# Iheckzza/FeatureMatching

Hardware: AMD Instinct MI355X
Metric: image-pairs/sec at 640x480 (coarse corr + dual-softmax mutual-NN + fine window refinement) (higher is better)
Workload: dtype i8 screening + f32 exact; 1 GPU; 640x480 pair, C=256 @1/8 (L=S=4800), Cf=64 @1/2, 5x5 fine window, 'peaky' descriptors; launch=hipGraph replay, concurrent_streams=4, fine_maps_layout=nchw

## Files before the change

### featurematching_amd/_lib.py

```python
from __future__ import annotations

import ctypes as C
import os

_HERE = os.path.dirname(os.path.abspath(__file__))
LIB_PATH = os.path.join(_HERE, "lib", "libfmatch_hip.so")

FM_OK = 0
FM_F32, FM_F16, FM_BF16 = 0, 1, 2
FM_E_UNSUPPORTED = -3
FM_E_CAPACITY = -5
FM_E_CANDIDATES = -6
FM_E_RANGE = -7
FM_E_DENSE = -8
FM_E_INTERNAL = -9
FM_E_STEP = -10
FM_DEV_RANGE = 4
FM_DEV_ALL_DENSE = 256
FM_MODE_EXACT_SCREENING, FM_MODE_DENSE, FM_MODE_NO_CELL_MAPS, FM_MODE_EXACT_STEP, FM_MODE_STATS = 1, 2, 4, 8, 16
FM_MODE_FLAT = 32
FM_MODE_ALONE = 64
FM_LOSS_CROSS_ENTROPY, FM_LOSS_FOCAL = 0, 1
FM_LAYOUT_NCHW_PREPARED = 2

_lib = None

_p = C.c_void_p
_i = C.c_int
_f = C.c_float

SIGNATURES = {
    "fm_version": (_i, []),
    "fm_strerror": (C.c_char_p, [_i]),
    "fm_default_cand_slots": (_i, [_f]),
    "fm_coarse_workspace_bytes": (_i, [_i, _i, _i, _i, _i, C.POINTER(C.c_size_t)]),
    "fm_coarse_workspace_bytes_mode": (_i, [_i, _i, _i, _i, _i, _i, _i, C.POINTER(C.c_size_t)]),
    "fm_coarse_match": (_i, [_p, _p, _i, _i, _i, _i, _i, _i, _i, _i, _f, _f, _i, _f, _p, _p,
                             _p, C.c_size_t, _i, _i, _p, _p, _p, _p, _p, _p, _i, _p, _p, _p]),
    "fm_coarse_match_dtype": (_i, [_p, _p, _i, _i, _i, _i, _i, _i, _i, _i, _i, _f, _f, _i, _f, _p, _p,
                                   _p, C.c_size_t, _i, _i, _p, _p, _p, _p, _p, _p, _i, _p, _p, _p]),
    "fm_coarse_match_maps": (_i, [_p, _p, _i, _i, _i, _i, _i, _i, _i, _i, _i, _f, _f, _i, _f, _p, _p,
                                  _p, C.c_size_t, _i, _i, _p, _p, _p, _p, _p, _p, _i, _p, _p, _p, _i, _i, _i, _i, _p, _p]),
    "fm_coarse_workspace_bytes_auto": (_i, [_i, _i, _i, _i, _i, C.POINTER(C.c_size_t)]),
    "fm_coarse_match_auto": (_i, [_p, _p, _i, _i, _i, _i, _i, _i, _i, _i, _i, _f, _f, _i, _f, _p, _p,
                                  _p, C.c_size_t, _i, _i, _p, _p, _p, _p, _p, _p, _i, _p, _p,
                                  C.POINTER(C.c_int32), C.POINTER(C.c_int32), C.POINTER(C.c_int32), _p]),
    "fm_debug_coarse_layout": (_i, [_i, _i, _i, _i, _i, C.POINTER(C.c_int64), _i]),
    "fm_debug_launch_corr": (_i, [_p, _i, _i, _i, _i, _i, _f, _f, _i, _p]),
    "fm_debug_launch_screen": (_i, [_p, _p, _p, _i, _i, _i, _i, _i, _f, _f, _p]),
    "fm_debug_launch_prep": (_i, [_p, _p, _p, _i, _i, _i, _i, _i, _p]),
    "fm_debug_launch_prep_f16": (_i, [_p, _p, _p, _i, _i, _i, _i, _i, _i, _p]),
    "fm_debug_reset_counters": (_i, [_p, _i, _i, _i, _i, _i, _p]),
    "fm_debug_unit_cert": (_i, [_i]),
    "fm_debug_unit_cert_layout": (_i, [_i, _i, _i, _i, _i, C.POINTER(C.c_int64), _i]),
    "fm_read_count": (_i, [_p, _i, C.POINTER(C.c_int32), _p]),
    "fm_read_count_info": (_i, [_p, _i, C.POINTER(C.c_int32), C.POINTER(C.c_int32), _p]),
    "fm_debug_launch_flat": (_i, [_p, _p, _p, _i, _i, _i, _i, _i, _f, _f, _i, _p]),
    "fm_coarse_softmax_stats": (_i, [_p, _i, _i, _i, _i, _i, C.POINTER(_p), C.POINTER(_p), C.POINTER(_i), C.POINTER(_p),
                                     C.POINTER(_p), C.POINTER(_i)]),
    "fm_dual_softmax_conf_at": (_i, [_p, _p, _i, _i, _i, _i, _f, _p, _p, _i, _p, _p, _i, _p, _p, _p, _i, _p, _p]),
    "fm_dual_softmax_backward_workspace_bytes": (C.c_size_t, [_i, _i, _i, _i]),
    "fm_dual_softmax_backward": (_i, [_p, _p, _i, _i, _i, _i, _f, _p, _p, _i, _p, _p, _i, _p, _p, _p, _p, _i, _p, C.c_size_t, _p,
                                      _p, _p]),
    "fm_dual_softmax_backward_dense": (_i, [_p, _p, _i, _i, _i, _i, _f, _p, _p, _i, _p, _p, _i, _p, _p, C.c_size_t, _p, _p, _p]),
    "fm_coarse_loss_workspace_bytes": (C.c_size_t, [_i, _i, _i, _i, _i]),
    "fm_coarse_loss_forward": (_i, [_p, _p, _i, _i, _i, _i, _f, _p, _p, _i, _p, _p, _i, _i, _f, _f, _f, _f, _p, _p, _p, _i, _p,
                                    C.c_size_t, _p, _p]),
    "fm_coarse_loss_backward": (_i, [_p, _p, _i, _i, _i, _i, _f, _p, _p, _i, _p, _p, _i, _i, _f, _f, _f, _f, _p, _p, _p, _i, _p,
                                     C.c_size_t, _p, _p, _p, _p]),
    "fm_supervise_workspace_bytes": (C.c_size_t, [_i, _i, _i, _i]),
    "fm_supervise_matches": (_i, [_p, _p, _i, _i, _i, _i, _i, _f, _p, C.c_size_t, _p, _p, _p, _p, _p, _p, _p, _p, _p, _p, _i, _p,
                                  _p]),
    "fm_fine_loss_workspace_bytes": (C.c_size_t, [_i]),
    "fm_fine_loss_forward": (_i, [_p, _p, _i, _p, _p, _i, _p, _p, C.c_size_t, _p, _p]),
    "fm_fine_loss_backward": (_i, [_p, _p, _i, _p, _p, _i, _p, C.c_size_t, _p, _p, _p, _p]),
    "fm_gather_windows": (_i, [_p, _i, _i, _i, _i, _i, _i, _i, _i, _i, _p, _p, _p, _i, _p, _p]),
    "fm_gather_windows_dtype": (_i, [_p, _i, _i, _i, _i, _i, _i, _i, _i, _i, _i, _p, _p, _p, _i, _p, _p]),
    "fm_coarse_cell_maps": (_i, [_p, _i, _i, _i, _i, _i, C.POINTER(_p), C.POINTER(_i), C.POINTER(_p),
                                 C.POINTER(_p), C.POINTER(_i), C.POINTER(_p)]),
    "fm_gather_windows_cells": (_i, [_p, _i, _i, _i, _i, _i, _i, _i, _i, _i, _p, _i, _p, _p, _p, _p, _i, _p, _p]),
    "fm_merge_pack_weights": (_i, [_p, _i, _p, _p]),
    "fm_gather_merge_windows": (_i, [_p, _i, _i, _i, _i, _i, _i, _i, _i, _i, _p, _i, _p, _p, _p, _p, _p, _p, _i, _p, _p]),
    "fm_gather_windows_pair": (_i, [_p, _p, _i, _i, _i, _i, _i, _i, _i, _i, _i, _i, _i, _i, _i, _p, _i, _p, _p, _i, _p,
                                    _p, _p, _p, _p, _p, _p, _p, _i, _p, _p, _p]),
    "fm_gather_merge_windows_nhwc": (_i, [_p, _p, _i, _i, _i, _i, _i, _i, _i, _i, _i, _i, _i, _i, _i, _i, _p, _p, _p, _p, _p,
                                          _p, _p, _i, _p, _p, _p]),
    "fm_coarse_tf_packed_bytes": (C.c_size_t, [_i]),
    "fm_coarse_tf_workspace_bytes": (_i, [_i, _i, _i, C.POINTER(C.c_size_t)]),
    "fm_coarse_tf_pack_weights": (_i, [_p, _i, _p, _p]),
    "fm_coarse_transformer": (_i, [_p, _p, _i, _i, _i, _i, _i, _p, _i, _p, _p, C.c_size_t, _p, _p, _p]),
    "fm_coarse_transformer_masked": (_i, [_p, _p, _p, _p, _i, _i, _i, _i, _i, _p, _i, _p, _p, C.c_size_t, _p, _p, _p]),
    "fm_fine_tf_packed_bytes": (C.c_size_t, []),
    "fm_fine_tf_pack_weights": (_i, [_p, _p, _p, _p]),
    "fm_fine_transformer": (_i, [_p, _p, _i, _p, _i, _i, _p, _p, _p, _p]),
    "fm_fine_transformer_status": (_i, [_p, _p, _i, _p, _i, _i, _p, _p, _p, _p, _p]),
    "fm_fine_transformer_start": (_i, [_p, _p, _i, _p, _i, _i, _p, _p, _p, _p, _i, _p, _p]),
    "fm_epipolar_errors": (_i, [_p, _p, _i, _p, _p, _i, _i, _p, _p, _p, _f, _p, _p, _p, _p]),
    "fm_fine_match": (_i, [_p, _p, _i, _p, _i, _i, _p, _p, _p, _p, _f, _p, _p, _p]),
    "fm_fine_match_backward_workspace_bytes": (C.c_size_t, [_i, _i]),
    "fm_fine_match_backward": (_i, [_p, _p, _i, _p, _i, _i, _p, _p, _f, _p, _p, _p, C.c_size_t, _p, _p, _p, _p, _p]),
    "fm_gather_windows_backward_workspace_bytes": (C.c_size_t, [_i, _i, _i, _i]),
    "fm_gather_windows_backward": (_i, [_p, _p, _p, _p, _i, _i, _i, _i, _i, _i, _i, _i, _i, _i, _i, _p, C.c_size_t, _p,
                                        _p]),
    "fm_fine_maps_scratch_bytes": (C.c_size_t, [_i, _i, _i, _i, _i, _i, _i]),
    "fm_fine_maps_scratch_bytes_dtype": (C.c_size_t, [_i, _i, _i, _i, _i, _i, _i, _i]),
    "fm_fine_match_maps_dtype": (_i, [_p, _p, _i, _i, _i, _i, _i, _i, _i, _i, _i, _i, _i, _i, _i, _p, _p, _p, _p, _i, _p, _p,
                                      _p, _p, _f, _p, _p, _p, _p]),
    "fm_fine_match_maps": (_i, [_p, _p, _i, _i, _i, _i, _i, _i, _i, _i, _i, _i, _i, _i, _p, _p, _p, _p, _i, _p, _p,
                                _p, _p, _f, _p, _p, _p, _p]),
}


class FMatchError(RuntimeError):
    def __init__(self, status: int, where: str):
        self.status = status
        msg = load().fm_strerror(status).decode()
        super().__init__(f"{where}: {msg} (status {status})")


DEBUG_SIGNATURES = {k: v for k, v in SIGNATURES.items() if k.startswith("fm_debug_")}
SIGNATURES = {k: v for k, v in SIGNATURES.items() if not k.startswith("fm_debug_")}
ALL_SIGNATURES = {**SIGNATURES, **DEBUG_SIGNATURES}


def load(path=None):
    global _lib
    if _lib is None:
        lib_path = path or LIB_PATH
        if not os.path.exists(lib_path):
            raise RuntimeError(
                f"{lib_path} is missing: the HIP library is the product and has no fallback. "
                "Build it with `make -C featurematching_amd/csrc` (hipcc, --offload-arch=gfx950).")
        import torch
        lib = C.CDLL(lib_path)
        for name, (res, args) in ALL_SIGNATURES.items():
            fn = getattr(lib, name)
            fn.restype = res
            fn.argtypes = args
        _lib = lib
    elif path is not None and os.path.abspath(path) != os.path.abspath(getattr(_lib, '_name', '')):
        raise RuntimeError("the library is already loaded; load an experimental build before any other use")
    return _lib


def check(status: int, where: str) -> None:
    if status != FM_OK:
        raise FMatchError(status, where)
```

### featurematching_amd/csrc/api.hip

```cpp
#include <math.h>
#include <stdlib.h>

#include "fm_debug.h"
#include "fm_internal.h"

namespace fm {

int g_unit_cert = 0;

int choose_splits(int N, int panels, int tiles, int target) {
  const int wg = N * panels;
#ifdef FM_TUNE_ENV
  if (const char* e = getenv("FM_TARGET_WGS")) target = atoi(e) > 0 ? atoi(e) : 256;
#endif
  int s = target / (wg > 0 ? wg : 1);
  if (s < 1) s = 1;
  const int smax = tiles / 2 > 0 ? tiles / 2 : 1;
  if (s > smax) s = smax;
  if (s > 32) s = 32;
  return s;
}

static int choose_screen_chunks(int N, int Lp, int nunits, int* units_per_chunk, bool alone) {
  const long nrb = (long)N * (Lp / 32);
  const int cu = nrb * ((nunits + 63) / 64) >= 1024 ? 64 : (alone && nrb * ((nunits + 7) / 8) <= 8192 ? 8 : 32);
  *units_per_chunk = cu;
  return (nunits + cu - 1) / cu;
}

constexpr int kMaxPassTarget = 256;
constexpr int kMaxPassSlots = 512;

CoarseWs coarse_layout(int N, int L, int S, int C, int slots, bool alone) {
  CoarseWs w{};
  C = padded_channels(C);
  w.N = N; w.L = L; w.S = S; w.C = C; w.slots = slots;
  w.Lp = round_up(L, kPanelRows);
  w.Sp = round_up(S, kTileCols);
  w.panels = w.Lp / kPanelRows;
  w.tiles = w.Sp / kTileCols;
  w.splits = choose_splits(N, w.panels, w.tiles);
  {
    int target = N * w.panels >= kMaxPassSlots ? 10 * kMaxPassSlots : (alone ? kMaxPassSlots : kMaxPassTarget);
    if (target == kMaxPassTarget && w.tiles / choose_splits(N, w.panels, w.tiles, kMaxPassTarget) >= 32) target = kMaxPassSlots;
    w.splits0 = choose_splits(N, w.panels, w.tiles, target);
    w.top2 = N * w.panels < kMaxPassSlots && w.tiles / choose_splits(N, w.panels, w.tiles, kMaxPassTarget) < 32;
  }
#ifdef FM_TUNE_ENV
  if (const char* e = getenv("FM_TARGET_WGS0")) w.splits0 = choose_splits(N, w.panels, w.tiles, atoi(e) > 0 ? atoi(e) : kMaxPassTarget);
#endif
  w.splits_s = choose_screen_chunks(N, w.Lp, w.Sp / 32, &w.units_s, alone);
  const size_t rows = (size_t)N * w.Lp, cols = (size_t)N * w.Sp;
  const size_t nblk = (rows * slots + 255) / 256;
  size_t o = 0;
  auto take = [&](auto& r, size_t count) { r.at = o; o = align256(o + r.bytes(count)); };
  auto since = [&](size_t at) { return Span{at, o - at}; };
  take(w.cand.count, rows);
  take(w.ccand.count, cols);
  take(w.cand_b.count, rows);
  take(w.ccand_b.count, cols);
  take(w.dense_cnt, N);
  w.counters[0] = since(w.cand.count.at);
  take(w.cell0, rows);
  take(w.cell1, cols);
  take(w.ties0, kTieCap + 1);
  take(w.ties1, kTieCap + 1);
  w.reassign[0] = since(w.cell0.at);
  take(w.rowmax_u, rows);
  take(w.colmax_u, cols);
  take(w.blocktot, nblk);
  w.reassign[1] = since(w.blocktot.at);
  take(w.scalars, 1);
  w.reassign[2] = Span{w.scalars.at, sizeof(Scalars::flags)};
  w.counters[1] = Span{w.scalars.at, sizeof(Scalars)};
  w.prep_zero = since(w.cand.count.at);
  take(w.q0, rows * C); take(w.q1, cols * C);
  take(w.sigimg, (size_t)N * 2);
  take(w.imgstat, (size_t)N * 8);
  take(w.l1_0, rows); take(w.l1_1, cols);
  take(w.bstat0, rows / 32); take(w.bstat1, cols / 32);
  take(w.emarg, N);
  take(w.nmr, rows); take(w.nmc, cols);
  take(w.umax, rows / 32 * (cols / N / 32));
  take(w.cand.idx, rows * slots); take(w.cand.x, rows * slots);
  take(w.ccand.idx, cols * slots); take(w.ccand.x, cols * slots);
  take(w.thr_r, rows); take(w.thr_c, cols);
  take(w.wmaxb, rows / 32); take(w.cmaxu, cols / 32);
  take(w.tmin_r, rows / 32); take(w.tmin_c, cols / 32);
  take(w.umax2, rows / 32 * (cols / N / 32));
  take(w.upos, rows / 32 * (cols / N / 32));
  w.common_total = o;
  take(w.hi0, rows * C); take(w.lo0, rows * C);
  take(w.hi1, cols * C); take(w.lo1, cols * C);
  take(w.f16inv, N);
  take(w.rowB, rows * w.splits); take(w.colB, cols * w.panels);
  take(w.rsum, rows); take(w.csum, cols);
  take(w.nmr2, rows); take(w.nmc2, cols);
  take(w.cand_b.idx, rows * slots); take(w.cand_b.x, rows * slots);
  take(w.ccand_b.idx, cols * slots); take(w.ccand_b.x, cols * slots);
  w.total = o;
  return w;
}

}

using namespace fm;

extern "C" int fm_version(void) { return FM_VERSION; }

extern "C" const char* fm_strerror(int s) {
  switch (s) {
    case FM_OK: return "ok";
    case FM_E_NULL: return "required pointer is NULL";
    case FM_E_SHAPE: return "inconsistent or non-positive shape";
    case FM_E_UNSUPPORTED: return "unsupported configuration (C % 4 == 0 and C <= 256, Cf = 64, W in {5,7}, thr in (0,1))";
    case FM_E_WORKSPACE: return "workspace too small or not 256-byte aligned";
    case FM_E_CAPACITY: return "more matches than the output capacity";
    case FM_E_CANDIDATES: return "a coarse row or column exceeded its candidate slots (FM_MODE_EXACT_SCREENING, then more cand_slots)";
    case FM_E_RANGE: return "descriptor not finite or |x| >= 32768, or similarities of several thousand (screening margin >= 2^60)";
    case FM_E_DENSE: return "flat similarity in a sample: call again with FM_MODE_DENSE";
    case FM_E_INTERNAL: return "assignment kernel: bounded wait for predecessor workgroups ran out; call again";
    case FM_E_STEP: return "int8 screening step too small for a descriptor outside the sampled rows: call again with FM_MODE_EXACT_STEP";
    default: return s > 0 ? hipGetErrorString((hipError_t)s) : "unknown fmatch status";
  }
}

extern "C" int fm_default_cand_slots(float thr) {
  if (!(thr > 0.f)) return 64;
  int need = (int)ceilf(1.0f / thr) + 3;
  int s = 8;
  while (s < need && s < 64) s <<= 1;
  return s;
}

static float inv_ct_of(int C, float temperature) { return 1.0f / ((float)C * temperature); }

static bool valid_slots(int s) { return s >= 4 && s <= 64 && (s & (s - 1)) == 0; }

constexpr int kKnownModes = FM_MODE_DENSE | FM_MODE_EXACT_SCREENING | FM_MODE_NO_CELL_MAPS | FM_MODE_EXACT_STEP | FM_MODE_STATS |
                            FM_MODE_FLAT | FM_MODE_ALONE;

static int check_coarse_shape(int N, int L, int S, int C, int cand_slots) {
  if (N <= 0 || L <= 0 || S <= 0) return FM_E_SHAPE;
  if (!valid_channels(C) || !valid_slots(cand_slots)) return FM_E_UNSUPPORTED;
  return FM_OK;
}

static int checked_layout(bool have_ptrs, int N, int L, int S, int C, int cand_slots, CoarseWs* w) {
  if (!have_ptrs) return FM_E_NULL;
  if (const int bad = check_coarse_shape(N, L, S, C, cand_slots)) return bad;
  *w = coarse_layout(N, L, S, C, cand_slots);
  return FM_OK;
}

struct CoarsePlan {
  bool alone;
  bool exact_step;
  bool flat;
  bool allow_dead;
  bool prep_f16;
  int f16_force;
  bool dense;
  float list_cap;
  bool reduce;
  bool rescreen;
  bool exact_lists;
  bool conf;
  bool cell_maps;
  SelectFlags select() const { return {rescreen, dense, cell_maps, reduce}; }
  size_t workspace_bytes(const CoarseWs& w) const { return dense ? w.total : w.common_total; }
};

static CoarsePlan plan_coarse(int mode, bool conf, int cand_slots) {
  const bool all_rows = conf || (mode & FM_MODE_STATS) != 0;
  CoarsePlan p;
  p.alone = (mode & FM_MODE_ALONE) != 0;
  p.exact_step = (mode & FM_MODE_EXACT_STEP) != 0;
  p.flat = (mode & FM_MODE_FLAT) != 0 && !all_rows;
  p.allow_dead = !all_rows;
  p.dense = all_rows || (mode & (FM_MODE_DENSE | FM_MODE_EXACT_SCREENING | FM_MODE_FLAT)) != 0;
  p.prep_f16 = p.dense && !p.flat;
  p.f16_force = (mode & FM_MODE_EXACT_SCREENING) ? 1 : (conf ? 2 : 0);
  p.list_cap = conf ? 0.1f : 1.f;
  p.rescreen = (mode & FM_MODE_EXACT_SCREENING) != 0;
  p.reduce = p.rescreen || all_rows || (p.flat && cand_slots > 8);
  p.exact_lists = all_rows;
  p.conf = conf;
  p.cell_maps = (mode & FM_MODE_NO_CELL_MAPS) == 0;
  return p;
}

extern "C" int fm_coarse_workspace_bytes_mode(int N, int L, int S, int C, int cand_slots, int mode, int want_conf_matrix,
                                              size_t* bytes) {
  CoarseWs w;
  if (const int bad = checked_layout(bytes != nullptr, N, L, S, C, cand_slots, &w)) return bad;
  if (mode & ~kKnownModes) return FM_E_UNSUPPORTED;
  *bytes = plan_coarse(mode, want_conf_matrix != 0, cand_slots).workspace_bytes(w);
  return FM_OK;
}

extern "C" int fm_coarse_workspace_bytes(int N, int L, int S, int C, int cand_slots, size_t* bytes) {
  return fm_coarse_workspace_bytes_mode(N, L, S, C, cand_slots, FM_MODE_DENSE | FM_MODE_EXACT_SCREENING, 1, bytes);
}

extern "C" int fm_debug_coarse_layout(int N, int L, int S, int C, int cand_slots, int64_t* out, int n_out) {
  if (!out) return FM_E_NULL;
  if (n_out < 40) return FM_E_SHAPE;
  CoarseWs w;
  if (const int bad = checked_layout(true, N, L, S, C, cand_slots, &w)) return bad;
  const auto at = [](const auto& r) { return (int64_t)r.at; };
  const int64_t v[41] = {w.N, w.L, w.S, w.C, w.Lp, w.Sp, w.panels, w.tiles, w.splits, w.slots,
                         at(w.cand.count), at(w.ccand.count), at(w.scalars), at(w.blocktot), at(w.hi0), at(w.lo0),
                         at(w.hi1), at(w.lo1), at(w.q0), at(w.q1), at(w.sigimg), at(w.l1_0), at(w.nmr), at(w.nmr),
                         at(w.rowB), at(w.colB), at(w.nmr), at(w.nmc), at(w.rsum), at(w.csum), at(w.cand.idx),
                         at(w.cand.x), at(w.ccand.idx), at(w.umax), at(w.dense_cnt), at(w.rowmax_u), at(w.colmax_u),
                         w.splits_s, w.units_s, (int64_t)w.total, (int64_t)w.common_total};
  for (int i = 0; i < 40; ++i) out[i] = v[i];
  if (n_out > 40) out[40] = v[40];
  return FM_OK;
}

template <int K>
static hipError_t clear_spans(char* base, const Span (&spans)[K], hipStream_t st) {
  for (const Span& s : spans) {
    const hipError_t e = hipMemsetAsync(base + s.at, 0, s.bytes, st);
    if (e != hipSuccess) return e;
  }
  return hipSuccess;
}

static int coarse_match_impl(const CoarseCall& c, const MapCopyJob* job, bool resume) {
  if (!c.feat0 || !c.feat1 || !c.workspace || !c.d_count) return FM_E_NULL;
  if (c.in_dtype != FM_F32 && c.in_dtype != FM_F16 && c.in_dtype != FM_BF16) return FM_E_UNSUPPORTED;
  if (c.cap > 0 && (!c.b_ids || !c.i_ids || !c.j_ids || !c.mkpts0_c || !c.mkpts1_c || !c.mconf)) return FM_E_NULL;
  if (c.cap < 0 || c.L != c.h0c * c.w0c || c.S != c.h1c * c.w1c) return FM_E_SHAPE;
  if (const int bad = check_coarse_shape(c.N, c.L, c.S, c.C, c.cand_slots)) return bad;
  if (!(c.thr > 0.f) || !(c.thr < 1.f) || !(c.temperature > 0.f)) return FM_E_UNSUPPORTED;
  if (c.mode & ~kKnownModes) return FM_E_UNSUPPORTED;
  const CoarsePlan p = plan_coarse(c.mode, c.conf_matrix != nullptr, c.cand_slots);
  const CoarseWs w = coarse_layout(c.N, c.L, c.S, c.C, c.cand_slots, p.alone);
  if (c.workspace_bytes < p.workspace_bytes(w) || ((uintptr_t)c.workspace & 255)) return FM_E_WORKSPACE;
  char* base = (char*)c.workspace;
  hipStream_t st = (hipStream_t)c.stream;
  const float inv_ct = inv_ct_of(c.C, c.temperature);
  const float thr_list = fminf(c.thr, p.list_cap);
#define FM_TRY(call) do { const hipError_t e_ = (call); if (e_ != hipSuccess) return (int)e_; } while (0)
  if (!resume) {
    FM_TRY(launch_prep(c.feat0, c.feat1, c.in_dtype, c.C, w, base, p.exact_step, p.flat, st));
    FM_TRY(launch_max_i8(w, base, unit_cert_on(w, !p.dense), st));
    if (p.flat) FM_TRY(launch_stab(w, base, inv_ct, c.thr, p.allow_dead, st));
    else FM_TRY(launch_screen(c.feat0, c.feat1, c.in_dtype, c.C, w, base, inv_ct, c.thr, p.dense, p.allow_dead, st));
  } else {
    FM_TRY(clear_spans(base, w.reassign, st));
  }
  if (p.prep_f16) FM_TRY(launch_prep_f16(c.feat0, c.feat1, c.in_dtype, c.C, w, base, p.f16_force, st));
  if (p.dense) FM_TRY(launch_dense(w, base, inv_ct, thr_list, st));
  if (p.reduce) FM_TRY(launch_reduce(w, base, inv_ct, st));
  if (p.rescreen) FM_TRY(launch_dense(w, base, inv_ct, thr_list, st, nullptr, 1));
  if (p.exact_lists) FM_TRY(launch_exact_lists(w, base, inv_ct, c.feat0, c.feat1, c.in_dtype, c.C, st));
  if (p.conf) {
    FM_TRY(launch_dense(w, base, inv_ct, c.thr, st, c.conf_matrix));
    FM_TRY(launch_conf_patch(w, base, inv_ct, c.conf_matrix, st));
  }
#undef FM_TRY
  return (int)launch_select(w, base, c, inv_ct, p.select(), job);
}

extern "C" int fm_coarse_match(const float* feat0, const float* feat1, int N, int L, int S, int C, int h0c, int w0c,
                               int h1c, int w1c, float temperature, float thr, int border_rm, float scale_px,
                               const float* scale0, const float* scale1, void* workspace, size_t workspace_bytes,
                               int cand_slots, int mode, int64_t* b_ids, int64_t* i_ids, int64_t* j_ids,
                               float* mkpts0_c, float* mkpts1_c, float* mconf, int cap, int32_t* d_count,
                               float* conf_matrix, void* stream) {
  const CoarseCall c{feat0, feat1, FM_F32, N, L, S, C, h0c, w0c, h1c, w1c, temperature, thr, border_rm, scale_px, scale0, scale1,
                     workspace, workspace_bytes, cand_slots, mode, b_ids, i_ids, j_ids, mkpts0_c, mkpts1_c, mconf, cap,
                     d_count, conf_matrix, stream};
  return coarse_match_impl(c, nullptr, false);
}

extern "C" int fm_coarse_match_dtype(const void* feat0, const void* feat1, int in_dtype, int N, int L, int S, int C,
                                     int h0c, int w0c, int h1c, int w1c, float temperature, float thr, int border_rm,
                                     float scale_px, const float* scale0, const float* scale1, void* workspace,
                                     size_t workspace_bytes, int cand_slots, int mode, int64_t* b_ids,
                                     int64_t* i_ids, int64_t* j_ids, float* mkpts0_c, float* mkpts1_c, float* mconf,
                                     int cap, int32_t* d_count, float* conf_matrix, void* stream) {
  const CoarseCall c{feat0, feat1, in_dtype, N, L, S, C, h0c, w0c, h1c, w1c, temperature, thr, border_rm, scale_px, scale0,
                     scale1, workspace, workspace_bytes, cand_slots, mode, b_ids, i_ids, j_ids, mkpts0_c, mkpts1_c, mconf, cap,
                     d_count, conf_matrix, stream};
  return coarse_match_impl(c, nullptr, false);
}

extern "C" int fm_coarse_match_maps(const void* feat0, const void* feat1, int in_dtype, int N, int L, int S, int C,
                                    int h0c, int w0c, int h1c, int w1c, float temperature, float thr, int border_rm,
                                    float scale_px, const float* scale0, const float* scale1, void* workspace,
                                    size_t workspace_bytes, int cand_slots, int mode, int64_t* b_ids,
                                    int64_t* i_ids, int64_t* j_ids, float* mkpts0_c, float* mkpts1_c, float* mconf,
                                    int cap, int32_t* d_count, float* conf_matrix, const float* feat_f1, int Nf, int Cf,
                                    int Hf1, int Wf1, void* scratch1, void* stream) {
  if (!feat_f1 || !scratch1) return FM_E_NULL;
  if (Nf <= 0 || Hf1 <= 0 || Wf1 <= 0) return FM_E_SHAPE;
  if (Cf != 64) return FM_E_UNSUPPORTED;
  if (((uintptr_t)scratch1 & 15) || ((uintptr_t)feat_f1 & 15)) return FM_E_WORKSPACE;
  const MapCopyJob job{feat_f1, (float*)scratch1, Nf, Hf1, Wf1};
  const CoarseCall c{feat0, feat1, in_dtype, N, L, S, C, h0c, w0c, h1c, w1c, temperature, thr, border_rm, scale_px, scale0,
                     scale1, workspace, workspace_bytes, cand_slots, mode, b_ids, i_ids, j_ids, mkpts0_c, mkpts1_c, mconf, cap,
                     d_count, conf_matrix, stream};
  return coarse_match_impl(c, &job, false);
}

constexpr int kAutoDataModes = FM_MODE_DENSE | FM_MODE_EXACT_SCREENING | FM_MODE_EXACT_STEP | FM_MODE_FLAT;

extern "C" int fm_coarse_workspace_bytes_auto(int N, int L, int S, int C, int max_cand_slots, size_t* bytes) {
  if (max_cand_slots == 0) max_cand_slots = 64;
  return fm_coarse_workspace_bytes(N, L, S, C, max_cand_slots, bytes);
}

extern "C" int fm_coarse_match_auto(const void* feat0, const void* feat1, int in_dtype, int N, int L, int S, int C,
                                    int h0c, int w0c, int h1c, int w1c, float temperature, float thr, int border_rm,
                                    float scale_px, const float* scale0, const float* scale1, void* workspace,
                                    size_t workspace_bytes, int max_cand_slots, int mode, int64_t* b_ids, int64_t* i_ids,
                                    int64_t* j_ids, float* mkpts0_c, float* mkpts1_c, float* mconf, int cap,
                                    int32_t* d_count, float* conf_matrix, int32_t* hint_io, int32_t* m_out,
                                    int32_t* info_out, void* stream) {
  if (!m_out) return FM_E_NULL;
  if (max_cand_slots == 0) max_cand_slots = 64;
  if (!valid_slots(max_cand_slots)) return FM_E_UNSUPPORTED;
  if (mode & ~kKnownModes) return FM_E_UNSUPPORTED;
  if (!(thr > 0.f) || !(thr < 1.f)) return FM_E_UNSUPPORTED;
  const int slots0 = fm_default_cand_slots(thr) < max_cand_slots ? fm_default_cand_slots(thr) : max_cand_slots;
  const int fixed = mode & ~kAutoDataModes;
  const bool full_stats = conf_matrix != nullptr || (mode & FM_MODE_STATS) != 0;
  int cur = mode & kAutoDataModes;
  if (full_stats) cur |= FM_MODE_EXACT_SCREENING;
  int slots = slots0;
  if (conf_matrix && slots < 16 && max_cand_slots >= 16) slots = 16;
  const int slots_start = slots;
  if (hint_io && *hint_io) {
    cur |= *hint_io & kAutoDataModes;
    const int hs = (*hint_io >> 8) & 0xff;
    if (valid_slots(hs) && hs <= max_cand_slots && hs > slots) slots = hs;
  }
  bool tried_wide = slots > slots0, retried_internal = false;
  int st = FM_OK;
  int32_t m = 0, info = 0;
  int attempts = 0;
  CoarseCall c{feat0, feat1, in_dtype, N, L, S, C, h0c, w0c, h1c, w1c, temperature, thr, border_rm, scale_px, scale0, scale1,
               workspace, workspace_bytes, slots, mode, b_ids, i_ids, j_ids, mkpts0_c, mkpts1_c, mconf, cap, d_count,
               conf_matrix, stream};
  for (int attempt = 0; attempt < 10; ++attempt) {
    ++attempts;
    const int call_mode = fixed | cur | ((cur & FM_MODE_FLAT) ? FM_MODE_DENSE : 0);
    c.cand_slots = slots; c.mode = call_mode;
    st = coarse_match_impl(c, nullptr, false);
    if (st != FM_OK) return st;
    st = fm_read_count_info(d_count, cap, &m, &info, stream);
    if (st == FM_E_DENSE && !(cur & FM_MODE_DENSE) && !conf_matrix && !(mode & FM_MODE_STATS)) {
      cur |= FM_MODE_DENSE;
      if ((info & ~FM_DEV_ALL_DENSE) != FM_DEV_DENSE) continue;
      c.mode = fixed | cur;
      st = coarse_match_impl(c, nullptr, true);
      if (st != FM_OK) return st;
      st = fm_read_count_info(d_count, cap, &m, &info, stream);
    }
    if (st == FM_OK) break;
    if (st == FM_E_STEP && !(cur & FM_MODE_EXACT_STEP)) { cur |= FM_MODE_EXACT_STEP; continue; }
    if (st == FM_E_DENSE && !(cur & FM_MODE_DENSE)) { cur |= FM_MODE_DENSE; continue; }
    if (st == FM_E_CANDIDATES && (cur & FM_MODE_DENSE) && !tried_wide && slots < 16 && max_cand_slots >= 16 &&
        !(cur & FM_MODE_EXACT_SCREENING)) {
      slots = 16; cur |= FM_MODE_EXACT_STEP; tried_wide = true;
      continue;
    }
    if (st == FM_E_CANDIDATES && !(cur & FM_MODE_EXACT_SCREENING)) {
      if (tried_wide) slots = slots0;
      cur |= FM_MODE_EXACT_SCREENING | FM_MODE_DENSE;
      continue;
    }
    if (st == FM_E_CANDIDATES && slots < max_cand_slots) { slots *= 2; continue; }
    if (st == FM_E_INTERNAL && !retried_internal) { retried_internal = true; continue; }
    break;
  }
  *m_out = m;
  if (info_out) *info_out = info;
  if (hint_io && (st == FM_OK || st == FM_E_CAPACITY)) {
    int learnt = cur & kAutoDataModes;
    if (full_stats) learnt &= ~FM_MODE_EXACT_SCREENING | (mode & FM_MODE_EXACT_SCREENING);
    if ((learnt & FM_MODE_DENSE) && !full_stats) {
      if (info & FM_DEV_ALL_DENSE) learnt |= FM_MODE_FLAT; else learnt &= ~FM_MODE_FLAT;
    }
    *hint_io = learnt | (slots != slots_start ? slots << 8 : 0) | (slots << 16) | (attempts << 24);
  }
  return st;
}

extern "C" int fm_coarse_cell_maps(void* workspace, int N, int L, int S, int C, int cand_slots, int32_t** cell0,
                                   int* pitch0, int32_t** ties0, int32_t** cell1, int* pitch1, int32_t** ties1) {
  CoarseWs w;
  if (const int bad = checked_layout(workspace && cell0 && cell1 && pitch0 && pitch1 && ties0 && ties1, N, L, S, C,
                                     cand_slots, &w))
    return bad;
  *cell0 = w.cell0.in(workspace); *pitch0 = w.Lp; *ties0 = w.ties0.in(workspace);
  *cell1 = w.cell1.in(workspace); *pitch1 = w.Sp; *ties1 = w.ties1.in(workspace);
  return FM_OK;
}

extern "C" int fm_coarse_softmax_stats(void* workspace, int N, int L, int S, int C, int cand_slots, const float** nm_r,
                                       const float** sum_r, int* pitch_r, const float** nm_c, const float** sum_c,
                                       int* pitch_c) {
  CoarseWs w;
  if (const int bad = checked_layout(workspace && nm_r && sum_r && pitch_r && nm_c && sum_c && pitch_c, N, L, S, C,
                                     cand_slots, &w))
    return bad;
  *nm_r = w.nmr.in(workspace); *sum_r = w.rsum.in(workspace); *pitch_r = w.Lp;
  *nm_c = w.nmc.in(workspace); *sum_c = w.csum.in(workspace); *pitch_c = w.Sp;
  return FM_OK;
}

extern "C" int fm_debug_launch_corr(void* workspace, int N, int L, int S, int C, int cand_slots, float temperature,
                                    float thr, int mode, void* stream) {
  CoarseWs w;
  if (const int bad = checked_layout(workspace, N, L, S, C, cand_slots, &w)) return bad;
  if (mode < 0 || mode > 2) return FM_E_UNSUPPORTED;
  hipStream_t st = (hipStream_t)stream;
  if (mode == 0) return (int)launch_max_i8(w, (char*)workspace, unit_cert_on(w), st);
  if (mode == 1) return (int)launch_dense(w, (char*)workspace, inv_ct_of(C, temperature), thr, st);
  return (int)launch_dense(w, (char*)workspace, inv_ct_of(C, temperature), thr, st, nullptr, 1);
}

extern "C" int fm_debug_launch_screen(void* workspace, const float* feat0, const float* feat1, int N, int L, int S,
                                          int C, int cand_slots, float temperature, float thr, void* stream) {
  CoarseWs w;
  if (const int bad = checked_layout(workspace && feat0 && feat1, N, L, S, C, cand_slots, &w)) return bad;
  return (int)launch_screen(feat0, feat1, FM_F32, C, w, (char*)workspace, inv_ct_of(C, temperature), thr, 1, 1,
                                (hipStream_t)stream);
}

extern "C" int fm_debug_launch_prep(void* workspace, const float* feat0, const float* feat1, int N, int L, int S, int C,
                                    int cand_slots, void* stream) {
  CoarseWs w;
  if (const int bad = checked_layout(workspace && feat0 && feat1, N, L, S, C, cand_slots, &w)) return bad;
  return (int)launch_prep(feat0, feat1, FM_F32, C, w, (char*)workspace, 0, 0, (hipStream_t)stream);
}

extern "C" int fm_debug_launch_prep_f16(void* workspace, const float* feat0, const float* feat1, int N, int L, int S,
                                        int C, int cand_slots, int force, void* stream) {
  CoarseWs w;
  if (const int bad = checked_layout(workspace && feat0 && feat1, N, L, S, C, cand_slots, &w)) return bad;
  return (int)launch_prep_f16(feat0, feat1, FM_F32, C, w, (char*)workspace, force, (hipStream_t)stream);
}

extern "C" int fm_debug_launch_flat(void* workspace, const float* feat0, const float* feat1, int N, int L, int S, int C,
                                    int cand_slots, float temperature, float thr, int which, void* stream) {
  CoarseWs w;
  if (const int bad = checked_layout(workspace && feat0 && feat1, N, L, S, C, cand_slots, &w)) return bad;
  if (which < 0 || which > 1) return FM_E_UNSUPPORTED;
  if (which == 0) return (int)launch_prep(feat0, feat1, FM_F32, C, w, (char*)workspace, 0, 1, (hipStream_t)stream);
  return (int)launch_stab(w, (char*)workspace, inv_ct_of(C, temperature), thr, 1, (hipStream_t)stream);
}

extern "C" int fm_debug_reset_counters(void* workspace, int N, int L, int S, int C, int cand_slots, void* stream) {
  CoarseWs w;
  if (const int bad = checked_layout(workspace, N, L, S, C, cand_slots, &w)) return bad;
  return (int)clear_spans((char*)workspace, w.counters, (hipStream_t)stream);
}

extern "C" int fm_debug_unit_cert(int mode) {
  const int prev = g_unit_cert;
  if (mode >= 0 && mode <= 2) g_unit_cert = mode;
  return prev;
}

extern "C" int fm_debug_unit_cert_layout(int N, int L, int S, int C, int cand_slots, int64_t* out, int n_out) {
  if (!out) return FM_E_NULL;
  if (n_out < 9) return FM_E_SHAPE;
  CoarseWs w;
  if (const int bad = checked_layout(true, N, L, S, C, cand_slots, &w)) return bad;
  const int64_t v[9] = {(int64_t)w.umax.at, (int64_t)w.umax2.at, (int64_t)w.upos.at, (int64_t)w.thr_r.at, (int64_t)w.thr_c.at,
                        (int64_t)w.tmin_r.at, (int64_t)w.tmin_c.at, (int64_t)(w.scalars.at + offsetof(Scalars, cert_units)), w.top2};
  for (int i = 0; i < 9; ++i) out[i] = v[i];
  return FM_OK;
}

extern "C" int fm_read_count(const int32_t* d_count, int cap, int32_t* m_out, void* stream) {
  return fm_read_count_info(d_count, cap, m_out, nullptr, stream);
}

extern "C" int fm_read_count_info(const int32_t* d_count, int cap, int32_t* m_out, int32_t* info_out, void* stream) {
  if (!d_count || !m_out) return FM_E_NULL;
  int32_t h[2] = {0, 0};
  hipStream_t st = (hipStream_t)stream;
  hipError_t e = hipMemcpyAsync(h, d_count, sizeof(h), hipMemcpyDeviceToHost, st);
  if (e != hipSuccess) return (int)e;
  e = hipStreamSynchronize(st);
  if (e != hipSuccess) return (int)e;
  *m_out = h[0];
  if (info_out) *info_out = h[1];
  if (h[1] & FM_DEV_INTERNAL) return FM_E_INTERNAL;
  if (h[1] & FM_DEV_RANGE) return FM_E_RANGE;
  if (h[1] & FM_DEV_STEP) return FM_E_STEP;
  if (h[1] & FM_DEV_DENSE) return FM_E_DENSE;
  if (h[1] & FM_DEV_CANDIDATES) return FM_E_CANDIDATES;
  if (h[1] & FM_DEV_CAPACITY) return FM_E_CAPACITY;
  if (h[0] > cap) return FM_E_CAPACITY;
  return FM_OK;
}
```

### featurematching_amd/csrc/coarse_screen.hip

```cpp
#include <stdlib.h>
#include <string.h>

#include <type_traits>

#include "fm_device.h"
#include "fm_wave_device.h"

namespace fm {

constexpr int kMaxExact = 24;

struct ScreenArgs {
  const signed char* q0; const signed char* q1;
  const void* src0; const void* src1; int c_in, in_dtype;
  const unsigned* rowmax_u; const unsigned* colmax_u;
  const float* sigimg;
  const float* imgstat;
  const float* l1_0; const float* l1_1;
  const float4* bstat0; const float4* bstat1;
  const float* umax;
  float* nmr; float* nmc; float* emarg;
  int* dense_cnt; Scalars* scal;
  int* rcount; int* rlist_j; float* rlist_x;
  int* ccount; int* clist_i; float* clist_x;
  int L, S, Lp, Sp, slots, dense_enabled;
  int allow_dead;
  float k, lt, inv_ct, cpad;
};

__device__ __forceinline__ int sig_threshold(float nm, float emu, float inv_kss) {
  const float t = floorf((-kSkipLog2 - emu - nm) * inv_kss) - 1.f;
  return (int)fminf(fmaxf(t, -1.0e9f), 1.0e9f);
}

__global__ __launch_bounds__(256) void k_stab(ScreenArgs a, float* f16inv) {
  const int side = blockIdx.z, b = blockIdx.y;
  const int len = side ? a.S : a.L, lenp = side ? a.Sp : a.Lp;
  const int idx = blockIdx.x * 256 + threadIdx.x;
  const float sig0 = a.sigimg[b * 2], sig1 = a.sigimg[b * 2 + 1];
  const float* ist = a.imgstat + (long)b * 8;
  const float l1A_max = ist[0], clipA = ist[1], infA = ist[2], l1B_max = ist[3], clipB = ist[4], infB = ist[5];
  const float ss = sig0 * sig1;
  if (blockIdx.x == 0 && side == 0 && threadIdx.x == 0) {
    const float emarg = margin_log2(q8_margin_raw(sig0, l1A_max, clipA, sig1, l1B_max, clipB, a.cpad), a.inv_ct);
    a.emarg[b] = emarg;
    const bool clipped = clipA > 0.f || clipB > 0.f;
    const float sc0 = f16_plane_scale(127.f * sig0), sc1 = f16_plane_scale(127.f * sig1);
    f16inv[b] = (1.0f / sc0) * (1.0f / sc1);
    if (!(l1A_max < INFINITY) || !(l1B_max < INFINITY)) atomicOr(&a.scal->flags, (unsigned)FM_DEV_RANGE);
    else if (!(emarg < 60.f)) atomicOr(&a.scal->flags, (unsigned)(clipped ? FM_DEV_STEP : FM_DEV_RANGE));
    else if (!(infA * sc0 < 65504.f) || !(infB * sc1 < 65504.f)) atomicOr(&a.scal->flags, (unsigned)FM_DEV_STEP);
    a.dense_cnt[b] = 1;
    a.scal->dense_units = 1;
  }
  if (idx >= lenp) return;
  const long g = (long)b * lenp + idx;
  float nm = -INFINITY;
  if (idx < len) {
    const float ln2 = 0.69314718f;
    const float l1 = (side ? a.l1_1 : a.l1_0)[g];
    const unsigned mx = (side ? a.colmax_u : a.rowmax_u)[g];
    const bool dead = a.allow_dead && 2.002f * l1 * (side ? infA : infB) * a.inv_ct + 1e-3f <
                                          (a.lt + __builtin_log2f((float)(side ? a.L : a.S))) * ln2;
    const float mraw = side ? q8_margin_raw(sig0, l1A_max, clipA, sig1, l1, clipB, a.cpad)
                            : q8_margin_raw(sig0, l1, clipA, sig1, l1B_max, clipB, a.cpad);
    nm = dead ? -INFINITY : neg_stabiliser_log2(ss * q_decode(mx), mraw, a.inv_ct);
  }
  (side ? a.nmc : a.nmr)[g] = nm;
}

struct RowsExtra {
  int* thr_r; int* thr_c; float* wmaxb; float* cmaxu;
  int* tmin_r; int* tmin_c;
  const int* umax2; const int* upos;
  int look;
  int count_cert;
  int nchunks, chunk_units, items;
};

__global__ __launch_bounds__(256) void k_thresh(ScreenArgs a, RowsExtra x) {
  const int side = blockIdx.z, b = blockIdx.y;
  const int len = side ? a.S : a.L, lenp = side ? a.Sp : a.Lp;
  const int idx = blockIdx.x * 256 + threadIdx.x;
  const int lane = threadIdx.x & 63;
  const float sig0 = a.sigimg[b * 2], sig1 = a.sigimg[b * 2 + 1];
  const float* ist = a.imgstat + (long)b * 8;
  const float l1A_max = ist[0], clipA = ist[1], infA = ist[2], l1B_max = ist[3], clipB = ist[4], infB = ist[5];
  const float ss = sig0 * sig1;
  const float kss = a.k * ss;
  const bool screen_ok = kss > 1e-30f && kss < 1e30f;
  const float inv_kss = screen_ok ? 1.0f / kss : 0.f;
  if (blockIdx.x == 0 && side == 0 && threadIdx.x == 0) {
    const float emarg = margin_log2(q8_margin_raw(sig0, l1A_max, clipA, sig1, l1B_max, clipB, a.cpad), a.inv_ct);
    a.emarg[b] = emarg;
    const bool clipped = clipA > 0.f || clipB > 0.f;
    const float emarg0 = margin_log2(q8_margin_raw(sig0, l1A_max, 0.f, sig1, l1B_max, 0.f, a.cpad), a.inv_ct);
    if (!(l1A_max < INFINITY) || !(l1B_max < INFINITY)) atomicOr(&a.scal->flags, (unsigned)FM_DEV_RANGE);
    else if (!(emarg < 60.f)) atomicOr(&a.scal->flags, (unsigned)(clipped ? FM_DEV_STEP : FM_DEV_RANGE));
    else if (clipped && emarg > 2.0f * emarg0 + 1.0f) atomicOr(&a.scal->flags, (unsigned)FM_DEV_STEP);
  }
  if (idx >= lenp) return;
  const long g = (long)b * lenp + idx;
  const int blk = idx >> 5;
  const int nblk = lenp / 32;
  float nm = -INFINITY;
  float emu = 0.f;
  if (idx < len) {
    const float ln2 = 0.69314718f;
    const float l1 = (side ? a.l1_1 : a.l1_0)[g];
    const unsigned mx = (side ? a.colmax_u : a.rowmax_u)[g];
    const float bl1 = (side ? a.bstat1 : a.bstat0)[(long)b * nblk + blk].x;
    const bool dead = a.allow_dead && 2.002f * l1 * (side ? infA : infB) * a.inv_ct + 1e-3f <
                                          (a.lt + __builtin_log2f((float)(side ? a.L : a.S))) * ln2;
    const float mraw = side ? q8_margin_raw(sig0, l1A_max, clipA, sig1, l1, clipB, a.cpad)
                            : q8_margin_raw(sig0, l1, clipA, sig1, l1B_max, clipB, a.cpad);
    nm = dead ? -INFINITY : neg_stabiliser_log2(ss * q_decode(mx), mraw, a.inv_ct);
    emu = margin_log2(side ? q8_margin_raw(sig0, l1A_max, clipA, sig1, bl1, clipB, a.cpad)
                           : q8_margin_raw(sig0, bl1, clipA, sig1, l1B_max, clipB, a.cpad), a.inv_ct);
  }
  (side ? a.nmc : a.nmr)[g] = nm;
  const int thr = idx < len ? sig_threshold(nm, emu, inv_kss) : 0x3fffffff;
  (side ? x.thr_c : x.thr_r)[g] = thr;
  const float bm = half_all<OpMax>(nm);
  const int tm = half_all<OpMin>(thr);
  if ((lane & 31) == 0) {
    (side ? x.cmaxu : x.wmaxb)[(long)b * nblk + blk] = bm;
    (side ? x.tmin_c : x.tmin_r)[(long)b * nblk + blk] = tm;
  }
}

template <int C>
__global__ __launch_bounds__(256, 3) void k_screen_rows(ScreenArgs a, RowsExtra x) {
  constexpr int KS8 = C / 32;
  constexpr int LIST = 256;
  const int tid = threadIdx.x;
  const int lane = tid & 63;
  const int wv = __builtin_amdgcn_readfirstlane(tid >> 6);
  const int r = lane & 31, h = lane >> 5;
  __shared__ int s_list[4][LIST];

  const int nrb = a.Lp / 32, nunits = a.Sp / 32;
  const int item = xcd_contiguous(blockIdx.x, gridDim.x) * 4 + wv;
  if (item >= x.items) return;
  const int per_sample = nrb * x.nchunks;
  const int b = item / per_sample;
  int kk = item - b * per_sample;
  const int chunk = kk / nrb;
  const int rb = kk - chunk * nrb;
  const int wrow0 = rb * 32;
  if (wrow0 >= a.L) return;
  const int u0 = chunk * x.chunk_units;
  const int U = min(x.chunk_units, nunits - u0);

  const float sig0 = a.sigimg[b * 2], sig1 = a.sigimg[b * 2 + 1];
  const float* ist = a.imgstat + (long)b * 8;
  const float clipA = ist[1], clipB = ist[4];
  const float bl1A = a.bstat0[(long)b * nrb + rb].x;
  const float wmax = x.wmaxb[(long)b * nrb + rb];
  const int ul_c = min(lane, U - 1);
  const float um = a.umax[((long)b * nrb + rb) * nunits + u0 + ul_c];
  const float cm = x.cmaxu[(long)b * nunits + u0 + ul_c];
  const float bl1B = a.bstat1[(long)b * nunits + u0 + ul_c].x;
  const bool look = x.look && ist[6] != 0.f;
  const int um2 = x.umax2[((long)b * nrb + rb) * nunits + u0 + ul_c];
  const int upos = x.upos[((long)b * nrb + rb) * nunits + u0 + ul_c];
  const int tmin = min(x.tmin_r[(long)b * nrb + rb], x.tmin_c[(long)b * nunits + u0 + ul_c]);
  int trr[16];
  {
    const int* tp = x.thr_r + (long)b * a.Lp + wrow0 + 4 * h;
#pragma unroll
    for (int q = 0; q < 4; ++q) {
      const int4 t4 = *reinterpret_cast<const int4*>(tp + 8 * q);
      trr[4 * q] = t4.x; trr[4 * q + 1] = t4.y; trr[4 * q + 2] = t4.z; trr[4 * q + 3] = t4.w;
    }
  }
  v4i aq[KS8];
  {
    const signed char* src = a.q0 + (((long)b * a.Lp + wrow0) / 32 * KS8 * 64 + lane) * 16;
#pragma unroll
    for (int ks = 0; ks < KS8; ++ks) aq[ks] = *reinterpret_cast<const v4i*>(src + ks * 1024);
  }
  const float ss = sig0 * sig1;
  const float kss = a.k * ss;
  const bool screen_ok = kss > 1e-30f && kss < 1e30f;

  unsigned long long live;
  {
    const float emu = margin_log2(q8_margin_raw(sig0, bl1A, clipA, sig1, bl1B, clipB, a.cpad), a.inv_ct);
    const float top = __builtin_fmaf(um, kss, emu);
    const bool hot = lane < U && (!screen_ok || !((top + wmax < -kSkipLog2) && (top + cm < -kSkipLog2)));
    live = __ballot(hot);
  }
  const unsigned long long cert = look ? (live & __ballot(um2 <= tmin)) : 0ull;
  live &= ~cert;
  const bool flat = !screen_ok || a.dense_cnt[b] != 0;
  int nd_units = flat ? 1 : 0;
  int nlist = 0;
#ifdef FM_ABL_ROWS
  if (FM_ABL_ROWS & 1) live = 0;
#endif
  int cert_thr = 0x3fffffff, cert_key = 0;
  if (!flat && ((cert >> lane) & 1)) {
    const int g = upos & 15, lw = (upos >> 4) & 63;
    const int rl = (g & 3) + 8 * (g >> 2) + 4 * (lw >> 5), cl = lw & 31;
    cert_thr = min(x.thr_r[(long)b * a.Lp + wrow0 + rl], x.thr_c[(long)b * a.Sp + (u0 + lane) * 32 + cl]);
    cert_key = (lane << 10) | (rl << 5) | cl;
  }
  if (x.count_cert && cert && lane == 0) atomicAdd(&a.scal->cert_units, __builtin_popcountll(cert));
  if (!flat && live) {
    const bool row_edge = (wrow0 + 32 > a.L);
    const signed char* q1b = a.q1 + ((long)b * nunits + u0) * KS8 * 1024 + lane * 16;
    const int* tcb = x.thr_c + (long)b * a.Sp + u0 * 32 + r;
    auto load_unit = [&](int ul, v4i (&bq)[KS8], int& tcl) {
      const signed char* src = q1b + (long)ul * KS8 * 1024;
#pragma unroll
      for (int ks = 0; ks < KS8; ++ks) bq[ks] = *reinterpret_cast<const v4i*>(src + ks * 1024);
      tcl = tcb[ul * 32];
    };
    auto screen_unit = [&](int ul, const v4i (&bq)[KS8], int tcl) {
      const int ucol0 = (u0 + ul) * 32;
      v16i acc;
#pragma unroll
      for (int g = 0; g < 16; ++g) acc[g] = 0;
#pragma unroll
      for (int ks = 0; ks < KS8; ++ks) acc = __builtin_amdgcn_mfma_i32_32x32x32_i8(aq[ks], bq[ks], acc, 0, 0, 0);
      if (row_edge || ucol0 + 32 > a.S) {
        const bool cok = ucol0 + r < a.S;
#pragma unroll
        for (int g = 0; g < 16; ++g)
          if (!cok || wrow0 + (g & 3) + 8 * (g >> 2) + 4 * h >= a.L) acc[g] = kQMasked;
      }
      unsigned bm = 0;
#pragma unroll
      for (int g = 0; g < 16; ++g) bm |= (acc[g] > min(trr[g], tcl)) ? (1u << g) : 0u;
      unsigned long long hitl = __ballot(bm != 0);
      if (!hitl) return;
      int cnt = 0;
#pragma unroll
      for (int g = 0; g < 16; ++g) cnt += __builtin_popcountll(__ballot((bm >> g) & 1u));
      if (cnt > kMaxExact || nlist + cnt > LIST) { ++nd_units; return; }
      while (hitl) {
        const int l = __builtin_ctzll(hitl);
        hitl &= hitl - 1;
        unsigned bits = (unsigned)__builtin_amdgcn_readlane((int)bm, l);
        while (bits) {
          const int g = __builtin_ctz(bits);
          bits &= bits - 1;
          const int rl = (g & 3) + 8 * (g >> 2) + 4 * (l >> 5);
          if (lane == 0) s_list[wv][nlist] = (ul << 10) | (rl << 5) | (l & 31);
          ++nlist;
        }
      }
    };
    v4i bA[KS8], bB[KS8];
    int tcA = 0, tcB = 0;
    unsigned long long mask = live;
    int ulA = __builtin_ctzll(mask), ulB = -1;
    mask &= mask - 1;
    load_unit(ulA, bA, tcA);
    while (true) {
      ulB = -1;
      if (mask) { ulB = __builtin_ctzll(mask); mask &= mask - 1; load_unit(ulB, bB, tcB); }
      screen_unit(ulA, bA, tcA);
      if (ulB < 0 || nd_units) break;
      ulA = -1;
      if (mask) { ulA = __builtin_ctzll(mask); mask &= mask - 1; load_unit(ulA, bA, tcA); }
      screen_unit(ulB, bB, tcB);
      if (ulA < 0 || nd_units) break;
    }
  }
  if (!flat && cert && !nd_units) {
    const unsigned long long hits = __ballot((int)um > cert_thr);
    const int nh = __builtin_popcountll(hits);
    if (nlist + nh > LIST) ++nd_units;
    else {
      if ((hits >> lane) & 1) s_list[wv][nlist + __builtin_popcountll(hits & ((1ull << lane) - 1ull))] = cert_key;
      nlist += nh;
    }
  }
  if (nd_units) nlist = 0;

  int overflow = 0;
#ifdef FM_ABL_ROWS
  if (FM_ABL_ROWS & 2) nlist = 0;
#endif
  {
    constexpr int NPASS = 4;
    const int sub = lane >> 4, l16 = lane & 15;
    const int vpr = a.c_in >> 2;
    for (int e0 = 0; e0 < nlist; e0 += 4 * NPASS) {
      int myres = 0;
      float my_nmr = 0.f, my_nmc = 0.f;
      if (lane < 4 * NPASS && e0 + lane < nlist) {
        const int ky = s_list[wv][e0 + lane];
        const int row = wrow0 + ((ky >> 5) & 31), col = (u0 + ((ky >> 10) & 63)) * 32 + (ky & 31);
        const int pr = atomicAdd(&a.rcount[(long)b * a.Lp + row], 1);
        const int pc = atomicAdd(&a.ccount[(long)b * a.Sp + col], 1);
        my_nmr = a.nmr[(long)b * a.Lp + row];
        my_nmc = a.nmc[(long)b * a.Sp + col];
        myres = min(pr, 0xffff) | (min(pc, 0xffff) << 16);
      }
      int key[NPASS];
      float xs[NPASS];
#pragma unroll
      for (int h2 = 0; h2 < NPASS; h2 += 2) {
        float4 av[2][4], bv[2][4];
#pragma unroll
        for (int pp = 0; pp < 2; ++pp) {
          const int p = h2 + pp;
          const int idx = e0 + 4 * p + sub;
          key[p] = s_list[wv][min(idx, nlist - 1)];
          const int row = wrow0 + ((key[p] >> 5) & 31), col = (u0 + ((key[p] >> 10) & 63)) * 32 + (key[p] & 31);
          const long ro = ((long)b * a.L + row) * a.c_in, co = ((long)b * a.S + col) * a.c_in;
#pragma unroll
          for (int q = 0; q < 4; ++q) {
            const int v4 = l16 + 16 * q;
            const bool in = v4 < vpr;
            const int vc = in ? v4 : 0;
            float4 ta, tb;
            if (a.in_dtype == FM_F32) {
              ta = reinterpret_cast<const float4*>((const float*)a.src0 + ro)[vc];
              tb = reinterpret_cast<const float4*>((const float*)a.src1 + co)[vc];
            } else {
              ta = half4_to_float4(reinterpret_cast<const uint2*>((const unsigned short*)a.src0 + ro)[vc], a.in_dtype);
              tb = half4_to_float4(reinterpret_cast<const uint2*>((const unsigned short*)a.src1 + co)[vc], a.in_dtype);
            }
            av[pp][q] = in ? ta : make_float4(0.f, 0.f, 0.f, 0.f);
            bv[pp][q] = tb;
          }
        }
#pragma unroll
        for (int pp = 0; pp < 2; ++pp) {
          float sm = 0.f;
#pragma unroll
          for (int q = 0; q < 4; ++q) {
            sm = __builtin_fmaf(av[pp][q].x, bv[pp][q].x, sm);
            sm = __builtin_fmaf(av[pp][q].y, bv[pp][q].y, sm);
            sm = __builtin_fmaf(av[pp][q].z, bv[pp][q].z, sm);
            sm = __builtin_fmaf(av[pp][q].w, bv[pp][q].w, sm);
          }
          xs[h2 + pp] = row_sum16(sm);
        }
        if (e0 + 4 * (h2 + 2) >= nlist) break;
      }
#pragma unroll
      for (int p = 0; p < NPASS; ++p) {
        const int idx = e0 + 4 * p + sub;
        if (e0 + 4 * p >= nlist) break;
        const int pos = __shfl(myres, 4 * p + sub);
        const float nmr_e = __shfl(my_nmr, 4 * p + sub), nmc_e = __shfl(my_nmc, 4 * p + sub);
        if (l16 == 0 && idx < nlist) {
          const int row = wrow0 + ((key[p] >> 5) & 31), col = (u0 + ((key[p] >> 10) & 63)) * 32 + (key[p] & 31);
          const float rr = __builtin_fmaf(xs[p], a.k, nmr_e);
          const float cc = __builtin_fmaf(xs[p], a.k, nmc_e);
          const int pr = pos & 0xffff, pc = (pos >> 16) & 0xffff;
          const long grow = (long)b * a.Lp + row, gcol = (long)b * a.Sp + col;
          if (pr < a.slots) { a.rlist_j[grow * a.slots + pr] = col; a.rlist_x[grow * a.slots + pr] = rr > -kSkipLog2 ? xs[p] : -INFINITY; }
          else overflow = 1;
          if (pc < a.slots) { a.clist_i[gcol * a.slots + pc] = row; a.clist_x[gcol * a.slots + pc] = cc > -kSkipLog2 ? xs[p] : -INFINITY; }
          else overflow = 1;
        }
      }
    }
  }
  nd_units += __builtin_popcountll(__ballot(overflow != 0));
  if (nd_units && lane == 0) {
    a.dense_cnt[b] = 1;
    a.scal->dense_units = 1;
    if (!a.dense_enabled) atomicOr(&a.scal->flags, (unsigned)FM_DEV_DENSE);
  }
}

static void fill_screen_stats(ScreenArgs& a, const CoarseWs& w, char* base, float inv_ct, float thr, int allow_dead) {
  a.rowmax_u = w.rowmax_u.in(base); a.colmax_u = w.colmax_u.in(base);
  a.sigimg = w.sigimg.in(base); a.imgstat = w.imgstat.in(base);
  a.l1_0 = w.l1_0.in(base); a.l1_1 = w.l1_1.in(base);
  a.bstat0 = w.bstat0.in(base); a.bstat1 = w.bstat1.in(base);
  a.umax = w.umax.in(base);
  a.nmr = w.nmr.in(base); a.nmc = w.nmc.in(base); a.emarg = w.emarg.in(base);
  a.dense_cnt = w.dense_cnt.in(base); a.scal = w.scalars.in(base);
  a.L = w.L; a.S = w.S; a.Lp = w.Lp; a.Sp = w.Sp;
  a.slots = w.slots; a.allow_dead = allow_dead;
  a.k = inv_ct * kLog2e; a.lt = log2f(thr); a.inv_ct = inv_ct; a.cpad = (float)w.C;
}

hipError_t launch_stab(const CoarseWs& w, char* base, float inv_ct, float thr, int allow_dead, hipStream_t st) {
  ScreenArgs a;
  memset(&a, 0, sizeof(a));
  fill_screen_stats(a, w, base, inv_ct, thr, allow_dead);
  const int lenp = w.Lp > w.Sp ? w.Lp : w.Sp;
  hipLaunchKernelGGL(k_stab, dim3((lenp + 255) / 256, w.N, 2), dim3(256), 0, st, a, w.f16inv.in(base));
  return hipGetLastError();
}

hipError_t launch_screen(const void* feat0, const void* feat1, int in_dtype, int c_in, const CoarseWs& w, char* base,
                         float inv_ct, float thr, int dense_enabled, int allow_dead, hipStream_t st) {
  ScreenArgs a;
  memset(&a, 0, sizeof(a));
  fill_screen_stats(a, w, base, inv_ct, thr, allow_dead);
  a.in_dtype = in_dtype;
  a.q0 = w.q0.in(base); a.q1 = w.q1.in(base);
  a.src0 = feat0; a.src1 = feat1; a.c_in = c_in;
  a.rcount = w.cand.count.in(base); a.rlist_j = w.cand.idx.in(base); a.rlist_x = w.cand.x.in(base);
  a.ccount = w.ccand.count.in(base); a.clist_i = w.ccand.idx.in(base); a.clist_x = w.ccand.x.in(base);
  a.dense_enabled = dense_enabled;
  RowsExtra x;
  x.thr_r = w.thr_r.in(base); x.thr_c = w.thr_c.in(base);
  x.wmaxb = w.wmaxb.in(base); x.cmaxu = w.cmaxu.in(base);
  x.tmin_r = w.tmin_r.in(base); x.tmin_c = w.tmin_c.in(base);
  x.umax2 = w.umax2.in(base); x.upos = w.upos.in(base);
  x.look = g_unit_cert != 1;
  x.count_cert = g_unit_cert == 2;
  x.chunk_units = w.units_s;
  x.nchunks = w.splits_s;
#ifdef FM_TUNE_ENV
  if (const char* ev = getenv("FM_ROWS_CHUNK")) { x.chunk_units = atoi(ev); x.nchunks = (w.Sp / 32 + x.chunk_units - 1) / x.chunk_units; }
#endif
  x.items = (int)((long)w.N * (w.Lp / 32) * x.nchunks);
  const int lenp = w.Lp > w.Sp ? w.Lp : w.Sp;
  hipLaunchKernelGGL(k_thresh, dim3((lenp + 255) / 256, w.N, 2), dim3(256), 0, st, a, x);
  const int blocks_r = (x.items + 3) / 4;
  return with_padded_channels(w.C, [&](auto cc) {
    hipLaunchKernelGGL(k_screen_rows<cc.value>, dim3(blocks_r), dim3(256), 0, st, a, x);
    return hipGetLastError();
  });
}

}
```

### featurematching_amd/csrc/coarse_select.hip

```cpp
#include "fm_internal.h"
#include "fm_maps_device.h"

namespace fm {

struct SelArgs {
  const float* nmr; const float* nmc;
  const float* rowB; const float* colB;
  int exact;
  int cell_maps;
  int dense_enabled;
  const int* cand_count; const int* cand_j; const float* cand_x;
  const int* ccand_count; const int* ccand_i; const float* ccand_x;
  const int* cand_count_b; const int* cand_j_b; const float* cand_x_b;
  const int* ccand_count_b; const int* ccand_i_b; const float* ccand_x_b;
  const int* dense_cnt;
  const float* rsum; const float* csum;
  int sums_ready;
  int* blocktot; Scalars* scal;
  int N, L, S, C, Lp, Sp, splits, splits_s, panels, slots;
  int h0c, w0c, h1c, w1c, border;
  float k, thr, scale_px;
  const float* scale0; const float* scale1;
  int64_t* b_ids; int64_t* i_ids; int64_t* j_ids; float* k0; float* k1; float* mconf;
  int cap; int32_t* d_count;
  int* cell0; int* cell1;
  int* ties0; int* ties1;
  int nblk;
  MapCopyJob job;
  float* diag;
};

__device__ __forceinline__ bool interior(int id, int hh, int ww, int bd) {
  if (bd <= 0) return true;
  const int y = id / ww, x = id - y * ww;
  return y >= bd && y < hh - bd && x >= bd && x < ww - bd;
}

__device__ __forceinline__ float fold_partials(const float* p, int n, long pitch) {
  float t = 0.f;
  for (int q0 = 0; q0 < n; q0 += 32) {
    float v[32];
#pragma unroll
    for (int q = 0; q < 32; ++q) v[q] = p[(long)min(q0 + q, n - 1) * pitch];
#pragma unroll
    for (int q = 0; q < 32; ++q) t += (q0 + q < n) ? v[q] : 0.f;
  }
  return t;
}

__device__ __forceinline__ float list_sum(float e, int key, bool live, int slots, int base, int maxcnt) {
  if (maxcnt <= 1) return __shfl(live ? e : 0.f, base);
  int rank = 0;
  for (int q = 0; q < slots; ++q) {
    const int ok = __shfl(key, base + q);
    const int ol = __shfl(live ? 1 : 0, base + q);
    rank += (ol && ok < key) ? 1 : 0;
  }
  float t = 0.f;
  for (int rr = 0; rr < maxcnt; ++rr) {
    unsigned v = (live && rank == rr) ? __float_as_uint(e) : 0u;
    for (int m = 1; m < slots; m <<= 1) v |= (unsigned)__shfl_xor((int)v, m);
    t += __uint_as_float(v);
  }
  return t;
}

__device__ __forceinline__ float entry_conf(float x, float k, float nmr, float rs, float nmc, float cs) {
#pragma clang fp contract(off)
  const float pr = __builtin_amdgcn_exp2f(__builtin_fmaf(x, k, nmr)) / rs;
  const float pc = __builtin_amdgcn_exp2f(__builtin_fmaf(x, k, nmc)) / cs;
  return pr * pc;
}

__global__ __launch_bounds__(256) void k_select(SelArgs a) {
  __shared__ int sm[4];
  __shared__ int rowoff[64], rowcnt[64];
  __shared__ int s_kj[256];
  __shared__ float s_kc[256];
#ifdef FM_DIAG_CLOCK
  unsigned long long dg[6];
  dg[0] = __builtin_amdgcn_s_memrealtime();
#define SEL_STAMP(i) dg[i] = __builtin_amdgcn_s_memrealtime();
#else
#define SEL_STAMP(i)
#endif
  if ((int)blockIdx.x >= a.nblk) {
    __shared__ float tr_tile[64 * 65];
    nchw_to_nhwc64_units<float>(a.job.src, a.job.dst, a.job.Hf, a.job.Wf, a.job.N, tr_tile, (long)blockIdx.x - a.nblk,
                                (long)gridDim.x - a.nblk);
    return;
  }
  const int blk = blockIdx.x;
  SEL_STAMP(1)
  const int lane = threadIdx.x & 63;
  const long gid = (long)blk * 256 + threadIdx.x;
  const long grow = gid / a.slots;
  const int slot = (int)(gid - grow * a.slots);
  const int b = (int)(grow / a.Lp);
  const int i = (int)(grow - (long)b * a.Lp);
  const bool dense = a.dense_enabled && b < a.N && a.dense_cnt[b] > 0;
  const int* cand_count = dense ? a.cand_count_b : a.cand_count;
  const int* cand_j = dense ? a.cand_j_b : a.cand_j;
  const float* cand_x = dense ? a.cand_x_b : a.cand_x;
  const int* ccand_count = dense ? a.ccand_count_b : a.ccand_count;
  const int* ccand_i = dense ? a.ccand_i_b : a.ccand_i;
  const float* ccand_x = dense ? a.ccand_x_b : a.ccand_x;
  const bool row_ok = b < a.N && i < a.L;
  const long grow_c = row_ok ? grow : 0;
  const int b_c = row_ok ? b : 0, i_c = row_ok ? i : 0;
  const int base = lane - slot;
  auto group_sum = [&](float v) {
    float t = 0.f;
    for (int q = 0; q < a.slots; ++q) t += __shfl(v, base + q);
    return t;
  };
  auto share = [&](const float* p, int n, long pitch) {
    float t = 0.f;
    for (int q = slot; q < n; q += a.slots) t += p[(long)q * pitch];
    return t;
  };
  auto wave_max_int = [&](int v) {
#pragma unroll
    for (int m = 32; m >= 1; m >>= 1) v = max(v, __shfl_xor(v, m));
    return v;
  };
  auto row_denominator = [&](int row, float nm) {
    const long g = (long)b_c * a.Lp + row;
    if (dense) return a.sums_ready ? a.rsum[g] : group_sum(share(a.rowB + (long)b_c * a.splits * a.Lp + row, a.splits, a.Lp));
    const int c2 = min(cand_count[g], a.slots);
    const int k2 = cand_j[g * a.slots + slot];
    const float x2 = cand_x[g * a.slots + slot];
    return list_sum(__builtin_amdgcn_exp2f(__builtin_fmaf(x2, a.k, nm)), k2, slot < c2, a.slots, base, wave_max_int(c2));
  };
  const int cnt_raw = cand_count[grow_c];
  const int j_raw = cand_j[grow_c * a.slots + slot];
  const float x_raw = cand_x[grow_c * a.slots + slot];
  const float nmr_i = a.nmr[grow_c];
  const int cnt = row_ok ? min(cnt_raw, a.slots) : 0;
  const bool live = slot < cnt;
  float rs;
  if (dense) rs = a.sums_ready ? a.rsum[grow_c] : group_sum(share(a.rowB + (long)b_c * a.splits * a.Lp + i_c, a.splits, a.Lp));
  else rs = list_sum(__builtin_amdgcn_exp2f(__builtin_fmaf(x_raw, a.k, nmr_i)), j_raw, live, a.slots, base, wave_max_int(cnt));
  bool keep = false;
  int j = live ? j_raw : 0x7fffffff;
  float conf = 0.f, colbest = 0.f;
  if (dense && a.sums_ready) {
    for (int t0 = 0; t0 < a.slots; t0 += 4) {
      if (!__any(t0 < cnt)) break;
      bool act[4];
      int jt[4], ccnt[4], ci[4];
      float xt[4], nmc[4], cs[4], cx[4], nm2_l[4], rs2_l[4];
#pragma unroll
      for (int q = 0; q < 4; ++q) {
        const int t = t0 + q;
        act[q] = t < cnt;
        jt[q] = act[q] ? __shfl(j_raw, base + (t & (a.slots - 1))) : 0;
        xt[q] = __shfl(x_raw, base + (t & (a.slots - 1)));
        const long gcol = (long)b_c * a.Sp + jt[q];
        nmc[q] = a.nmc[gcol];
        ccnt[q] = ccand_count[gcol];
        ci[q] = ccand_i[gcol * a.slots + slot];
        cx[q] = ccand_x[gcol * a.slots + slot];
        cs[q] = a.csum[gcol];
      }
#pragma unroll
      for (int q = 0; q < 4; ++q) {
        ccnt[q] = act[q] ? min(ccnt[q], a.slots) : 0;
        const long g2 = (long)b_c * a.Lp + ((act[q] && slot < ccnt[q]) ? ci[q] : i_c);
        nm2_l[q] = a.nmr[g2];
        rs2_l[q] = a.rsum[g2];
      }
#pragma unroll
      for (int q = 0; q < 4; ++q) {
        const float ct = act[q] ? entry_conf(xt[q], a.k, nmr_i, rs, nmc[q], cs[q]) : 0.f;
        float cb = 0.f;
        const int cmax = wave_max_int(ccnt[q]);
        for (int e = 0; e < cmax; ++e) {
          const bool ea = e < ccnt[q];
          const int i2 = ea ? __shfl(ci[q], base + e) : i_c;
          const float x2 = __shfl(cx[q], base + e);
          const float nm2 = __shfl(nm2_l[q], base + e), rs2 = __shfl(rs2_l[q], base + e);
          const float c2 = entry_conf(x2, a.k, nm2, rs2, nmc[q], cs[q]);
          if (ea && i2 != i) cb = fmaxf(cb, c2);
          if (ea && i2 == i) cb = fmaxf(cb, ct);
        }
        if (act[q] && slot == t0 + q) { conf = ct; colbest = cb; }
      }
    }
  } else
  for (int t = 0; t < a.slots; ++t) {
    if (!__any(t < cnt)) break;
    const bool act = t < cnt;
    const int jt = act ? __shfl(j_raw, base + t) : 0;
    const float xt = __shfl(x_raw, base + t);
    const long gcol = (long)b_c * a.Sp + jt;
    const float nmc = a.nmc[gcol];
    const int ccnt = act ? min(ccand_count[gcol], a.slots) : 0;
    const int ci = ccand_i[gcol * a.slots + slot];
    const float cx = ccand_x[gcol * a.slots + slot];
    float cs;
    if (dense) cs = a.sums_ready ? a.csum[gcol] : group_sum(share(a.colB + (long)b_c * a.panels * a.Sp + jt, a.panels, a.Sp));
    else cs = list_sum(__builtin_amdgcn_exp2f(__builtin_fmaf(cx, a.k, nmc)), ci, slot < ccnt, a.slots, base, wave_max_int(ccnt));
    const bool col_sig = dense || __builtin_fmaf(xt, a.k, nmc) > -kSkipLog2;
    const float ct = (act && col_sig) ? entry_conf(xt, a.k, nmr_i, rs, nmc, cs) : 0.f;
    float cb = 0.f;
    const int cmax = wave_max_int(ccnt);
    for (int e = 0; e < cmax; ++e) {
      const bool ea = e < ccnt;
      const int i2 = ea ? __shfl(ci, base + e) : i_c;
      const float x2 = __shfl(cx, base + e);
      const bool other = ea && i2 != i;
      if (__any(other)) {
        const int i2c = other ? i2 : i_c;
        const float nm2 = a.nmr[(long)b_c * a.Lp + i2c];
        const float rs2 = row_denominator(i2c, nm2);
        const float c2 = entry_conf(x2, a.k, nm2, rs2, nmc, cs);
        if (other && (dense || __builtin_fmaf(x2, a.k, nm2) > -kSkipLog2)) cb = fmaxf(cb, c2);
      }
      if (ea && i2 == i) cb = fmaxf(cb, ct);
    }
    if (act && slot == t) { conf = ct; colbest = cb; }
  }
  float rowbest = conf;
  for (int m = 1; m < a.slots; m <<= 1) rowbest = fmaxf(rowbest, __shfl_xor(rowbest, m));
#ifdef FM_DIAG_CLOCK
  asm volatile("s_waitcnt vmcnt(0)" ::: "memory");
  SEL_STAMP(2)
#endif
  if (live)
    keep = conf > a.thr && conf == rowbest && conf == colbest &&
           interior(i, a.h0c, a.w0c, a.border) && interior(j, a.h1c, a.w1c, a.border);
  const int kj = keep ? j : 0x7fffffff;
  int rank = 0, nkeep = 0;
  for (int s = 0; s < a.slots; ++s) {
    const int oj = __shfl(kj, base + s);
    rank += (oj < kj) ? 1 : 0;
    nkeep += (oj != 0x7fffffff) ? 1 : 0;
  }
  const int q = threadIdx.x / a.slots;
  if (keep) { s_kj[q * a.slots + rank] = j; s_kc[q * a.slots + rank] = conf; }
  if (slot == 0) rowcnt[q] = nkeep;
  int tot = (slot == 0) ? nkeep : 0;
#pragma unroll
  for (int m = 32; m >= 1; m >>= 1) tot += __shfl_xor(tot, m);
  if (lane == 0) sm[threadIdx.x >> 6] = tot;
  __syncthreads();
  const int total = sm[0] + sm[1] + sm[2] + sm[3];
  if (threadIdx.x == 0)
    __hip_atomic_store(&a.blocktot[blk], total | (int)0x40000000, __ATOMIC_RELAXED, __HIP_MEMORY_SCOPE_AGENT);
  SEL_STAMP(3)
  int pre = 0;
  int polls = 0;
  for (int k = threadIdx.x; k < blk; k += 256) {
    int v;
    do {
      v = __hip_atomic_load(&a.blocktot[k], __ATOMIC_RELAXED, __HIP_MEMORY_SCOPE_AGENT);
      if (!(v & 0x40000000)) {
        if (++polls > (1 << 22)) { atomicOr(&a.scal->flags, (unsigned)FM_INT_LOOKBACK_TIMEOUT); v = 0x40000000; }
        else __builtin_amdgcn_s_sleep(1);
      }
    } while (!(v & 0x40000000));
    pre += v & 0x3fffffff;
  }
#pragma unroll
  for (int m = 32; m >= 1; m >>= 1) pre += __shfl_xor(pre, m);
  __syncthreads();
  if (lane == 0) sm[threadIdx.x >> 6] = pre;
  __syncthreads();
  pre = sm[0] + sm[1] + sm[2] + sm[3];
  const int rows_per_block = 256 / a.slots;
  if (threadIdx.x < 64) {
    const int cntq = threadIdx.x < rows_per_block ? rowcnt[threadIdx.x] : 0;
    int incl = cntq;
#pragma unroll
    for (int d = 1; d < 64; d <<= 1) {
      const int o = __shfl_up(incl, d);
      if (lane >= d) incl += o;
    }
    if (threadIdx.x < rows_per_block) rowoff[threadIdx.x] = pre + incl - cntq;
    bool all_dense = false;
    if (blk == a.nblk - 1 && a.dense_enabled) {
      bool mine = true;
      for (int bb = threadIdx.x; bb < a.N; bb += 64) mine = mine && a.dense_cnt[bb] > 0;
      all_dense = __all(mine);
    }
    if (blk == a.nblk - 1 && threadIdx.x == 63) {
      const int run = pre + incl;
      a.d_count[0] = run;
      unsigned fl = __hip_atomic_load(&a.scal->flags, __ATOMIC_RELAXED, __HIP_MEMORY_SCOPE_AGENT);
      if (!a.exact && (fl & (unsigned)FM_INT_SCREEN_OVERFLOW)) fl |= (unsigned)FM_DEV_CANDIDATES;
      if (fl & (unsigned)FM_INT_LOOKBACK_TIMEOUT) fl |= (unsigned)FM_DEV_INTERNAL;
      a.d_count[1] = (int)((fl & (15u | (unsigned)FM_DEV_INTERNAL | (unsigned)FM_DEV_STEP) & ~(unsigned)FM_DEV_CAPACITY) |
                           (run > a.cap ? (unsigned)FM_DEV_CAPACITY : 0u) | (all_dense ? (unsigned)FM_DEV_ALL_DENSE : 0u));
    }
  }
  __syncthreads();
  SEL_STAMP(4)
#ifdef FM_DIAG_CLOCK
#define SEL_DIAG_OUT                                                                                  \
  if (threadIdx.x == 0) {                                                                             \
    SEL_STAMP(5)                                                                                      \
    for (int q2 = 0; q2 < 6; ++q2) a.diag[blk * 8 + q2] = (float)(dg[q2] & 0xffffff);                 \
  }
#else
#define SEL_DIAG_OUT
#endif
  if (b >= a.N || slot >= rowcnt[q]) { SEL_DIAG_OUT return; }
  const long o = (long)rowoff[q] + slot;
  if (o >= a.cap) { SEL_DIAG_OUT return; }
  const int jj = s_kj[q * a.slots + slot];
  a.b_ids[o] = b; a.i_ids[o] = i; a.j_ids[o] = jj;
  if (a.cell_maps) {
    const int me = (int)o + 1;
    int old = atomicMax(&a.cell0[grow], me);
    int loser = old > me ? me : old;
    if (loser > 0) { const int p = atomicAdd(&a.ties0[0], 1); if (p < kTieCap) a.ties0[1 + p] = loser - 1; }
    old = atomicMax(&a.cell1[(long)b * a.Sp + jj], me);
    loser = old > me ? me : old;
    if (loser > 0) { const int p = atomicAdd(&a.ties1[0], 1); if (p < kTieCap) a.ties1[1 + p] = loser - 1; }
  }
  a.mconf[o] = s_kc[q * a.slots + slot];
  float s0x = a.scale_px, s0y = a.scale_px, s1x = a.scale_px, s1y = a.scale_px;
  if (a.scale0) { s0x = a.scale_px * a.scale0[b * 2]; s0y = a.scale_px * a.scale0[b * 2 + 1]; }
  if (a.scale1) { s1x = a.scale_px * a.scale1[b * 2]; s1y = a.scale_px * a.scale1[b * 2 + 1]; }
  a.k0[o * 2] = (float)(i % a.w0c) * s0x; a.k0[o * 2 + 1] = (float)(i / a.w0c) * s0y;
  a.k1[o * 2] = (float)(jj % a.w1c) * s1x; a.k1[o * 2 + 1] = (float)(jj / a.w1c) * s1y;
#ifdef FM_DIAG_CLOCK
  asm volatile("s_waitcnt vmcnt(0)" ::: "memory");
#endif
  SEL_DIAG_OUT
}

hipError_t launch_select(const CoarseWs& w, char* base, const CoarseCall& c, float inv_ct, SelectFlags flags,
                         const MapCopyJob* job) {
  SelArgs a;
  a.exact = flags.exact; a.dense_enabled = flags.dense; a.cell_maps = flags.cell_maps; a.sums_ready = flags.sums_ready;
  a.nmr = w.nmr.in(base); a.nmc = w.nmc.in(base);
  a.rowB = w.rowB.in(base); a.colB = w.colB.in(base);
  a.cand_count = w.cand.count.in(base); a.cand_j = w.cand.idx.in(base);
  a.cand_x = w.cand.x.in(base);
  a.ccand_count = w.ccand.count.in(base); a.ccand_i = w.ccand.idx.in(base);
  a.ccand_x = w.ccand.x.in(base);
  a.cand_count_b = w.cand_b.count.in(base); a.cand_j_b = w.cand_b.idx.in(base);
  a.cand_x_b = w.cand_b.x.in(base);
  a.ccand_count_b = w.ccand_b.count.in(base); a.ccand_i_b = w.ccand_b.idx.in(base);
  a.ccand_x_b = w.ccand_b.x.in(base);
  a.dense_cnt = w.dense_cnt.in(base);
  a.rsum = w.rsum.in(base); a.csum = w.csum.in(base);
  a.blocktot = w.blocktot.in(base);
  a.scal = w.scalars.in(base);
  a.N = w.N; a.L = w.L; a.S = w.S; a.C = w.C; a.Lp = w.Lp; a.Sp = w.Sp; a.splits = w.splits; a.splits_s = w.splits_s; a.panels = w.panels;
  a.slots = w.slots; a.h0c = c.h0c; a.w0c = c.w0c; a.h1c = c.h1c; a.w1c = c.w1c; a.border = c.border_rm;
  a.k = inv_ct * kLog2e; a.thr = c.thr; a.scale_px = c.scale_px; a.scale0 = c.scale0; a.scale1 = c.scale1;
  a.b_ids = c.b_ids; a.i_ids = c.i_ids; a.j_ids = c.j_ids; a.k0 = c.mkpts0_c; a.k1 = c.mkpts1_c; a.mconf = c.mconf;
  a.cap = c.cap; a.d_count = c.d_count;
  a.cell0 = w.cell0.in(base); a.cell1 = w.cell1.in(base);
  a.ties0 = w.ties0.in(base); a.ties1 = w.ties1.in(base);
  const int blocks = (int)(((long)w.N * w.Lp * w.slots + 255) / 256);
  a.nblk = blocks;
  a.diag = w.rowB.in(base);
  a.job = MapCopyJob{nullptr, nullptr, 0, 0, 0};
  int extra = 0;
  if (job && job->src) {
    a.job = *job;
    const long units = (long)((job->Wf + 63) / 64) * job->Hf * job->N;
    extra = (int)(units < 1024 ? units : 1024);
  }
  hipLaunchKernelGGL(k_select, dim3(blocks + extra), dim3(256), 0, (hipStream_t)c.stream, a);
  return hipGetLastError();
}

}
```

### featurematching_amd/csrc/fm_debug.h

```cpp
#ifndef FM_DEBUG_H_
#define FM_DEBUG_H_

#include "fmatch.h"

#ifdef __cplusplus
extern "C" {
#endif

int fm_debug_coarse_layout(int N, int L, int S, int C, int cand_slots, int64_t* out, int n_out);

int fm_debug_launch_corr(void* workspace, int N, int L, int S, int C, int cand_slots,
                         float temperature, float thr, int mode, void* stream);
int fm_debug_launch_screen(void* workspace, const float* feat0, const float* feat1, int N, int L, int S,
                               int C, int cand_slots, float temperature, float thr, void* stream);
int fm_debug_launch_prep(void* workspace, const float* feat0, const float* feat1, int N, int L, int S, int C,
                         int cand_slots, void* stream);
int fm_debug_launch_prep_f16(void* workspace, const float* feat0, const float* feat1, int N, int L, int S, int C,
                             int cand_slots, int force, void* stream);
int fm_debug_reset_counters(void* workspace, int N, int L, int S, int C, int cand_slots, void* stream);
int fm_debug_launch_flat(void* workspace, const float* feat0, const float* feat1, int N, int L, int S, int C,
                         int cand_slots, float temperature, float thr, int which, void* stream);
int fm_debug_unit_cert(int mode);
int fm_debug_unit_cert_layout(int N, int L, int S, int C, int cand_slots, int64_t* out, int n_out);

#ifdef __cplusplus
}
#endif
#endif
```

### featurematching_amd/csrc/fm_internal.h

```cpp
#pragma once
#include <hip/hip_runtime.h>
#include <stddef.h>
#include <stdint.h>

#include <type_traits>

#include "fmatch.h"

namespace fm {

constexpr int kPanelRows = 256;
constexpr int kTieCap = 1023;
constexpr int kTileCols = 64;
constexpr float kLog2e = 1.4426950408889634f;
constexpr float kSkipLog2 = 32.f;
constexpr unsigned FM_INT_SCREEN_OVERFLOW = 16u;
constexpr unsigned FM_INT_LOOKBACK_TIMEOUT = 64u;
constexpr int kPrepSampleRows = 32;
constexpr float kPrepHeadroom = 1.5f;

inline int round_up(int x, int m) { return (x + m - 1) / m * m; }
inline int padded_channels(int c) { return c <= 64 ? 64 : (c <= 128 ? 128 : 256); }
inline bool valid_channels(int c) { return c >= 4 && c <= 256 && c % 4 == 0; }
inline size_t align256(size_t x) { return (x + 255) & ~size_t(255); }

struct Span { size_t at, bytes; };
template <typename T>
inline T* span_ptr(void* base, const Span& s) { return reinterpret_cast<T*>(static_cast<char*>(base) + s.at); }
template <typename T>
struct Region {
  size_t at;
  T* in(void* base) const { return reinterpret_cast<T*>(static_cast<char*>(base) + at); }
  static size_t bytes(size_t count) { return count * sizeof(T); }
};
struct CandList { Region<int> count, idx; Region<float> x; };

template <int V> using int_c = std::integral_constant<int, V>;
template <typename F>
inline bool with_window(int W, F&& f) {
  if (W == 5) f(int_c<5>{});
  else if (W == 7) f(int_c<7>{});
  else return false;
  return true;
}

inline bool crop_shape_ok(int N, int Hf, int Wf, int stride, int m_max) {
  return N > 0 && Hf > 0 && Wf > 0 && stride > 0 && m_max >= 0;
}

struct Scalars {
  unsigned flags;
  int dense_units;
  int cert_units;
};

struct CoarseWs {
  int N, L, S, C, Lp, Sp, panels, tiles, splits, slots;
  int splits0;
  int splits_s, units_s;
  int top2;
  Span prep_zero;
  Span reassign[3];
  Span counters[2];
  CandList cand, ccand;
  CandList cand_b, ccand_b;
  Region<int> dense_cnt;
  Region<Scalars> scalars;
  Region<int> cell0, cell1;
  Region<int> ties0, ties1;
  Region<unsigned> rowmax_u, colmax_u;
  Region<int> blocktot;
  Region<signed char> q0, q1;
  Region<float> sigimg;
  Region<float> imgstat;
  Region<float> l1_0, l1_1;
  Region<float4> bstat0, bstat1;
  Region<float> emarg;
  Region<float> nmr, nmc;
  Region<float> umax;
  Region<int> thr_r, thr_c;
  Region<float> wmaxb, cmaxu;
  Region<int> tmin_r, tmin_c;
  Region<int> umax2, upos;
  size_t common_total;
  Region<_Float16> hi0, lo0, hi1, lo1;
  Region<float> f16inv;
  Region<float> rowB, colB;
  Region<float> rsum, csum;
  Region<float> nmr2, nmc2;
  size_t total;
};

int choose_splits(int N, int panels, int tiles, int target = 256);
CoarseWs coarse_layout(int N, int L, int S, int C, int slots, bool alone = false);

extern int g_unit_cert;
inline bool unit_cert_on(const CoarseWs& w, bool common_path = true) {
  return g_unit_cert == 2 || (g_unit_cert == 0 && w.top2 != 0 && common_path);
}

struct CoarseCall {
  const void *feat0, *feat1; int in_dtype;
  int N, L, S, C, h0c, w0c, h1c, w1c;
  float temperature, thr; int border_rm; float scale_px; const float *scale0, *scale1;
  void* workspace; size_t workspace_bytes;
  int cand_slots, mode;
  int64_t *b_ids, *i_ids, *j_ids; float *mkpts0_c, *mkpts1_c, *mconf; int cap; int32_t* d_count; float* conf_matrix;
  void* stream;
};

hipError_t launch_prep(const void* feat0, const void* feat1, int in_dtype, int c_in, const CoarseWs& w, char* base,
                       int exact_step, int planes, hipStream_t st);
hipError_t launch_stab(const CoarseWs& w, char* base, float inv_ct, float thr, int allow_dead, hipStream_t st);
hipError_t launch_prep_f16(const void* feat0, const void* feat1, int in_dtype, int c_in, const CoarseWs& w, char* base,
                           int force, hipStream_t st);
hipError_t launch_max_i8(const CoarseWs& w, char* base, bool top2, hipStream_t st);
hipError_t launch_dense(const CoarseWs& w, char* base, float inv_ct, float thr, hipStream_t st, float* conf = nullptr,
                        int rescreen = 0);
hipError_t launch_reduce(const CoarseWs& w, char* base, float inv_ct, hipStream_t st);
struct MapCopyJob {
  const float* src; float* dst; int N, Hf, Wf;
};
struct SelectFlags { bool exact, dense, cell_maps, sums_ready; };
hipError_t launch_select(const CoarseWs& w, char* base, const CoarseCall& c, float inv_ct, SelectFlags flags,
                         const MapCopyJob* job = nullptr);
hipError_t launch_conf_patch(const CoarseWs& w, char* base, float inv_ct, float* conf, hipStream_t st);
hipError_t launch_exact_lists(const CoarseWs& w, char* base, float inv_ct, const void* feat0, const void* feat1, int in_dtype,
                              int c_in, hipStream_t st);
hipError_t launch_screen(const void* feat0, const void* feat1, int in_dtype, int c_in, const CoarseWs& w, char* base,
                             float inv_ct, float thr, int dense_enabled, int allow_dead, hipStream_t st);

struct DsmBwdWs { Span v, u, sums, part; size_t total; };
inline DsmBwdWs dsm_bwd_layout(int N, int L, int S, int C) {
  DsmBwdWs w;
  w.v = {0, (size_t)N * L * 4};
  w.u = {w.v.bytes, (size_t)N * S * 4};
  w.sums = {0, w.v.bytes + w.u.bytes};
  w.part = {align256(w.sums.bytes), (size_t)4 * N * (size_t)(L > S ? L : S) * C * 4};
  w.total = w.part.at + w.part.bytes;
  return w;
}
struct DsmStats {
  const float *ofs_r, *sum_r; int pitch_r;
  const float *ofs_c, *sum_c; int pitch_c;
};
struct DsmProblem {
  const float *feat0, *feat1;
  int N, L, S, C;
  float k2, inv_ct;
  float *v, *u, *part;
};
int dsm_carve(const float* feat0, const float* feat1, int N, int L, int S, int C, float temperature, const DsmStats& s,
              void* workspace, size_t workspace_bytes, DsmProblem* p);
int dsm_begin(const float* feat0, const float* feat1, int N, int L, int S, int C, float temperature, const DsmStats& s,
              void* workspace, size_t workspace_bytes, hipStream_t st, DsmProblem* p);
int dsm_zsplit(int N, int R);
struct DsmSide { DsmProblem p; DsmStats s; };
inline DsmSide dsm_side(const DsmProblem& p, const DsmStats& s, int side) {
  if (!side) return {p, s};
  return {{p.feat1, p.feat0, p.N, p.S, p.L, p.C, p.k2, p.inv_ct, p.u, p.v, p.part},
          {s.ofs_c, s.sum_c, s.pitch_c, s.ofs_r, s.sum_r, s.pitch_r}};
}
inline dim3 dsm_sweep_grid(const DsmSide& o) { return dim3((o.p.L + 31) / 32, o.p.N, dsm_zsplit(o.p.N, o.p.L)); }
template <typename F>
inline hipError_t with_padded_channels(int C, F&& f) {
  const int Cp = padded_channels(C);
  return Cp == 64 ? f(int_c<64>{}) : Cp == 128 ? f(int_c<128>{}) : f(int_c<256>{});
}
hipError_t launch_sweep_combine(const DsmSide& o, int Z, const float* d_loss, float* d_out, hipStream_t st);
hipError_t launch_dsm_uv(const int64_t* b_ids, const int64_t* i_ids, const int64_t* j_ids, const float* gc, int K, int L, int S,
                         float* v, float* u, hipStream_t st);
hipError_t launch_dsm_entries(const DsmProblem& p, const int64_t* b_ids, const int64_t* i_ids, const int64_t* j_ids,
                              const float* gc, int K, float* d_feat0, float* d_feat1, hipStream_t st);

template <typename K>
inline hipError_t ensure_dynamic_lds(K kernel, int bytes, unsigned long long* done_mask) {
  int dev = 0;
  hipError_t e = hipGetDevice(&dev);
  if (e != hipSuccess) return e;
  const unsigned long long bit = 1ull << (dev & 63);
  if (__atomic_load_n(done_mask, __ATOMIC_ACQUIRE) & bit) return hipSuccess;
  e = hipFuncSetAttribute(reinterpret_cast<const void*>(kernel), hipFuncAttributeMaxDynamicSharedMemorySize, bytes);
  if (e == hipSuccess) __atomic_fetch_or(done_mask, bit, __ATOMIC_RELEASE);
  return e;
}

}
```

Before: 20450 image-pairs/s.

## Defer exact f32 dot products for certainly-surviving candidates to select kernel

```diff
diff --git a/featurematching_amd/_lib.py b/featurematching_amd/_lib.py
--- a/featurematching_amd/_lib.py
+++ b/featurematching_amd/_lib.py
@@ -53,6 +53,8 @@
     "fm_debug_reset_counters": (_i, [_p, _i, _i, _i, _i, _i, _p]),
     "fm_debug_unit_cert": (_i, [_i]),
     "fm_debug_unit_cert_layout": (_i, [_i, _i, _i, _i, _i, C.POINTER(C.c_int64), _i]),
+    "fm_debug_defer_exact": (_i, [_i]),
+    "fm_debug_defer_exact_layout": (_i, [_i, _i, _i, _i, _i, C.POINTER(C.c_int64), _i]),
     "fm_read_count": (_i, [_p, _i, C.POINTER(C.c_int32), _p]),
     "fm_read_count_info": (_i, [_p, _i, C.POINTER(C.c_int32), C.POINTER(C.c_int32), _p]),
     "fm_debug_launch_flat": (_i, [_p, _p, _p, _i, _i, _i, _i, _i, _f, _f, _i, _p]),
diff --git a/featurematching_amd/csrc/api.hip b/featurematching_amd/csrc/api.hip
--- a/featurematching_amd/csrc/api.hip
+++ b/featurematching_amd/csrc/api.hip
@@ -7,6 +7,7 @@
 namespace fm {
 
 int g_unit_cert = 0;
+int g_defer_exact = 0;
 
 int choose_splits(int N, int panels, int tiles, int target) {
   const int wg = N * panels;
@@ -167,7 +168,7 @@
   bool exact_lists;
   bool conf;
   bool cell_maps;
-  SelectFlags select() const { return {rescreen, dense, cell_maps, reduce}; }
+  SelectFlags select(bool deferred) const { return {rescreen, dense, cell_maps, reduce, deferred}; }
   size_t workspace_bytes(const CoarseWs& w) const { return dense ? w.total : w.common_total; }
 };
 
@@ -249,7 +250,8 @@
     FM_TRY(launch_prep(c.feat0, c.feat1, c.in_dtype, c.C, w, base, p.exact_step, p.flat, st));
     FM_TRY(launch_max_i8(w, base, unit_cert_on(w, !p.dense), st));
     if (p.flat) FM_TRY(launch_stab(w, base, inv_ct, c.thr, p.allow_dead, st));
-    else FM_TRY(launch_screen(c.feat0, c.feat1, c.in_dtype, c.C, w, base, inv_ct, c.thr, p.dense, p.allow_dead, st));
+    else FM_TRY(launch_screen(c.feat0, c.feat1, c.in_dtype, c.C, w, base, inv_ct, c.thr, p.dense, p.allow_dead,
+                              defer_exact_on(w, !p.dense), st));
   } else {
     FM_TRY(clear_spans(base, w.reassign, st));
   }
@@ -263,7 +265,7 @@
     FM_TRY(launch_conf_patch(w, base, inv_ct, c.conf_matrix, st));
   }
 #undef FM_TRY
-  return (int)launch_select(w, base, c, inv_ct, p.select(), job);
+  return (int)launch_select(w, base, c, inv_ct, p.select(defer_exact_on(w, resume || !p.dense)), job);
 }
 
 extern "C" int fm_coarse_match(const float* feat0, const float* feat1, int N, int L, int S, int C, int h0c, int w0c,
@@ -431,7 +433,7 @@
   CoarseWs w;
   if (const int bad = checked_layout(workspace && feat0 && feat1, N, L, S, C, cand_slots, &w)) return bad;
   return (int)launch_screen(feat0, feat1, FM_F32, C, w, (char*)workspace, inv_ct_of(C, temperature), thr, 1, 1,
-                                (hipStream_t)stream);
+                            defer_exact_on(w), (hipStream_t)stream);
 }
 
 extern "C" int fm_debug_launch_prep(void* workspace, const float* feat0, const float* feat1, int N, int L, int S, int C,
@@ -477,6 +479,23 @@
   const int64_t v[9] = {(int64_t)w.umax.at, (int64_t)w.umax2.at, (int64_t)w.upos.at, (int64_t)w.thr_r.at, (int64_t)w.thr_c.at,
                         (int64_t)w.tmin_r.at, (int64_t)w.tmin_c.at, (int64_t)(w.scalars.at + offsetof(Scalars, cert_units)), w.top2};
   for (int i = 0; i < 9; ++i) out[i] = v[i];
+  return FM_OK;
+}
+
+extern "C" int fm_debug_defer_exact(int mode) {
+  const int prev = g_defer_exact;
+  if (mode >= 0 && mode <= 2) g_defer_exact = mode;
+  return prev;
+}
+
+extern "C" int fm_debug_defer_exact_layout(int N, int L, int S, int C, int cand_slots, int64_t* out, int n_out) {
+  if (!out) return FM_E_NULL;
+  if (n_out < 3) return FM_E_SHAPE;
+  CoarseWs w;
+  if (const int bad = checked_layout(true, N, L, S, C, cand_slots, &w)) return bad;
+  out[0] = (int64_t)(w.scalars.at + offsetof(Scalars, defer_entries));
+  out[1] = 0x40000000;
+  out[2] = defer_exact_on(w) ? 1 : 0;
   return FM_OK;
 }
 
diff --git a/featurematching_amd/csrc/coarse_screen.hip b/featurematching_amd/csrc/coarse_screen.hip
--- a/featurematching_amd/csrc/coarse_screen.hip
+++ b/featurematching_amd/csrc/coarse_screen.hip
@@ -4,6 +4,7 @@
 #include <type_traits>
 
 #include "fm_device.h"
+#include "fm_exact_device.h"
 #include "fm_wave_device.h"
 
 namespace fm {
@@ -12,7 +13,7 @@
 
 struct ScreenArgs {
   const signed char* q0; const signed char* q1;
-  const void* src0; const void* src1; int c_in, in_dtype;
+  DescRows desc;
   const unsigned* rowmax_u; const unsigned* colmax_u;
   const float* sigimg;
   const float* imgstat;
@@ -31,6 +32,13 @@
 __device__ __forceinline__ int sig_threshold(float nm, float emu, float inv_kss) {
   const float t = floorf((-kSkipLog2 - emu - nm) * inv_kss) - 1.f;
   return (int)fminf(fmaxf(t, -1.0e9f), 1.0e9f);
+}
+
+__device__ __forceinline__ int sure_slack(float emarg, float kss, float k, float l1A_max, float infB) {
+#pragma clang fp contract(off)
+  const float P = k * l1A_max * infB;
+  const float dq = ceilf((2.0f * emarg + 7.62939453125e-6f * P + 0.01f) * (1.0f / kss) * 1.0001f);
+  return (emarg < 60.f && dq < 1.0e9f) ? (int)dq + 2 : 0x3fffffff;
 }
 
 __global__ __launch_bounds__(256) void k_stab(ScreenArgs a, float* f16inv) {
@@ -75,6 +83,8 @@
   const int* umax2; const int* upos;
   int look;
   int count_cert;
+  int defer;
+  int count_defer;
   int nchunks, chunk_units, items;
 };
 
@@ -138,6 +148,8 @@
   const int wv = __builtin_amdgcn_readfirstlane(tid >> 6);
   const int r = lane & 31, h = lane >> 5;
   __shared__ int s_list[4][LIST];
+  __shared__ int s_sure[4][LIST];
+  __shared__ int s_sq[4][LIST];
 
   const int nrb = a.Lp / 32, nunits = a.Sp / 32;
   const int item = xcd_contiguous(blockIdx.x, gridDim.x) * 4 + wv;
@@ -155,6 +167,8 @@
   const float sig0 = a.sigimg[b * 2], sig1 = a.sigimg[b * 2 + 1];
   const float* ist = a.imgstat + (long)b * 8;
   const float clipA = ist[1], clipB = ist[4];
+  const float l1A_max = ist[0], infB = ist[5];
+  const float emarg_b = a.emarg[b];
   const float bl1A = a.bstat0[(long)b * nrb + rb].x;
   const float wmax = x.wmaxb[(long)b * nrb + rb];
   const int ul_c = min(lane, U - 1);
@@ -165,7 +179,7 @@
   const int um2 = x.umax2[((long)b * nrb + rb) * nunits + u0 + ul_c];
   const int upos = x.upos[((long)b * nrb + rb) * nunits + u0 + ul_c];
   const int tmin = min(x.tmin_r[(long)b * nrb + rb], x.tmin_c[(long)b * nunits + u0 + ul_c]);
-  int trr[16];
+  v16i trr;
   {
     const int* tp = x.thr_r + (long)b * a.Lp + wrow0 + 4 * h;
 #pragma unroll
@@ -183,6 +197,7 @@
   const float ss = sig0 * sig1;
   const float kss = a.k * ss;
   const bool screen_ok = kss > 1e-30f && kss < 1e30f;
+  const int D = (x.defer && screen_ok) ? sure_slack(emarg_b, kss, a.k, l1A_max, infB) : 0x3fffffff;
 
   unsigned long long live;
   {
@@ -195,15 +210,17 @@
   live &= ~cert;
   const bool flat = !screen_ok || a.dense_cnt[b] != 0;
   int nd_units = flat ? 1 : 0;
-  int nlist = 0;
+  int nlist = 0, nsure = 0;
 #ifdef FM_ABL_ROWS
   if (FM_ABL_ROWS & 1) live = 0;
 #endif
-  int cert_thr = 0x3fffffff, cert_key = 0;
+  int cert_thr = 0x3fffffff, cert_tmx = 0x3fffffff, cert_key = 0;
   if (!flat && ((cert >> lane) & 1)) {
     const int g = upos & 15, lw = (upos >> 4) & 63;
     const int rl = (g & 3) + 8 * (g >> 2) + 4 * (lw >> 5), cl = lw & 31;
-    cert_thr = min(x.thr_r[(long)b * a.Lp + wrow0 + rl], x.thr_c[(long)b * a.Sp + (u0 + lane) * 32 + cl]);
+    const int tr = x.thr_r[(long)b * a.Lp + wrow0 + rl], tc = x.thr_c[(long)b * a.Sp + (u0 + lane) * 32 + cl];
+    cert_thr = min(tr, tc);
+    cert_tmx = max(tr, tc);
     cert_key = (lane << 10) | (rl << 5) | cl;
   }
   if (x.count_cert && cert && lane == 0) atomicAdd(&a.scal->cert_units, __builtin_popcountll(cert));
@@ -238,7 +255,7 @@
       int cnt = 0;
 #pragma unroll
       for (int g = 0; g < 16; ++g) cnt += __builtin_popcountll(__ballot((bm >> g) & 1u));
-      if (cnt > kMaxExact || nlist + cnt > LIST) { ++nd_units; return; }
+      if (cnt > kMaxExact || nlist + nsure + cnt > LIST) { ++nd_units; return; }
       while (hitl) {
         const int l = __builtin_ctzll(hitl);
         hitl &= hitl - 1;
@@ -247,8 +264,22 @@
           const int g = __builtin_ctz(bits);
           bits &= bits - 1;
           const int rl = (g & 3) + 8 * (g >> 2) + 4 * (l >> 5);
-          if (lane == 0) s_list[wv][nlist] = (ul << 10) | (rl << 5) | (l & 31);
-          ++nlist;
+          const int key = (ul << 10) | (rl << 5) | (l & 31);
+          int sure_e = 0, q_e = 0;
+          if (D != 0x3fffffff) {
+            int qv = acc[0], tv = trr[0];
+#pragma unroll
+            for (int g2 = 1; g2 < 16; ++g2) { qv = (g == g2) ? acc[g2] : qv; tv = (g == g2) ? trr[g2] : tv; }
+            const bool sure_l = min(tv, tcl) > -1000000000 && qv > max(tv, tcl) + D;
+            q_e = __builtin_amdgcn_readlane(qv, l);
+            sure_e = __builtin_amdgcn_readlane((int)sure_l, l);
+          }
+          if (lane == 0) {
+            if (sure_e) { s_sure[wv][nsure] = key; s_sq[wv][nsure] = q_e; }
+            else s_list[wv][nlist] = key;
+          }
+          nsure += sure_e;
+          nlist += 1 - sure_e;
         }
       }
     };
@@ -272,22 +303,47 @@
   if (!flat && cert && !nd_units) {
     const unsigned long long hits = __ballot((int)um > cert_thr);
     const int nh = __builtin_popcountll(hits);
-    if (nlist + nh > LIST) ++nd_units;
+    if (nlist + nsure + nh > LIST) ++nd_units;
     else {
-      if ((hits >> lane) & 1) s_list[wv][nlist + __builtin_popcountll(hits & ((1ull << lane) - 1ull))] = cert_key;
-      nlist += nh;
+      const unsigned long long sure = hits & __ballot(cert_thr > -1000000000 && (int)um > cert_tmx + D);
+      const unsigned long long rest = hits & ~sure, below = (1ull << lane) - 1ull;
+      if ((rest >> lane) & 1) s_list[wv][nlist + __builtin_popcountll(rest & below)] = cert_key;
+      if ((sure >> lane) & 1) {
+        s_sure[wv][nsure + __builtin_popcountll(sure & below)] = cert_key;
+        s_sq[wv][nsure + __builtin_popcountll(sure & below)] = (int)um;
+      }
+      nlist += __builtin_popcountll(rest);
+      nsure += __builtin_popcountll(sure);
     }
   }
-  if (nd_units) nlist = 0;
+  if (nd_units) nlist = nsure = 0;
 
   int overflow = 0;
+#ifdef FM_ABL_ROWS
+  if (FM_ABL_ROWS & 2) nsure = 0;
+#endif
+  for (int e0 = 0; e0 < nsure; e0 += 64) {
+    if (e0 + lane < nsure) {
+      const int ky = s_sure[wv][e0 + lane];
+      const float xq = ss * (float)s_sq[wv][e0 + lane];
+      const int row = wrow0 + ((ky >> 5) & 31), col = (u0 + ((ky >> 10) & 63)) * 32 + (ky & 31);
+      const long grow = (long)b * a.Lp + row, gcol = (long)b * a.Sp + col;
+      const int pr = atomicAdd(&a.rcount[grow], 1);
+      const int pc = atomicAdd(&a.ccount[gcol], 1);
+      if (pr < a.slots) { a.rlist_j[grow * a.slots + pr] = col | kDeferTag; a.rlist_x[grow * a.slots + pr] = xq; }
+      else overflow = 1;
+      if (pc < a.slots) { a.clist_i[gcol * a.slots + pc] = row | kDeferTag; a.clist_x[gcol * a.slots + pc] = xq; }
+      else overflow = 1;
+    }
+  }
+  if (x.count_defer && nsure && lane == 0) atomicAdd(&a.scal->defer_entries, nsure);
+
 #ifdef FM_ABL_ROWS
   if (FM_ABL_ROWS & 2) nlist = 0;
 #endif
   {
     constexpr int NPASS = 4;
     const int sub = lane >> 4, l16 = lane & 15;
-    const int vpr = a.c_in >> 2;
     for (int e0 = 0; e0 < nlist; e0 += 4 * NPASS) {
       int myres = 0;
       float my_nmr = 0.f, my_nmc = 0.f;
@@ -311,36 +367,10 @@
           const int idx = e0 + 4 * p + sub;
           key[p] = s_list[wv][min(idx, nlist - 1)];
           const int row = wrow0 + ((key[p] >> 5) & 31), col = (u0 + ((key[p] >> 10) & 63)) * 32 + (key[p] & 31);
-          const long ro = ((long)b * a.L + row) * a.c_in, co = ((long)b * a.S + col) * a.c_in;
-#pragma unroll
-          for (int q = 0; q < 4; ++q) {
-            const int v4 = l16 + 16 * q;
-            const bool in = v4 < vpr;
-            const int vc = in ? v4 : 0;
-            float4 ta, tb;
-            if (a.in_dtype == FM_F32) {
-              ta = reinterpret_cast<const float4*>((const float*)a.src0 + ro)[vc];
-              tb = reinterpret_cast<const float4*>((const float*)a.src1 + co)[vc];
-            } else {
-              ta = half4_to_float4(reinterpret_cast<const uint2*>((const unsigned short*)a.src0 + ro)[vc], a.in_dtype);
-              tb = half4_to_float4(reinterpret_cast<const uint2*>((const unsigned short*)a.src1 + co)[vc], a.in_dtype);
-            }
-            av[pp][q] = in ? ta : make_float4(0.f, 0.f, 0.f, 0.f);
-            bv[pp][q] = tb;
-          }
+          exact_dot16_load(a.desc, b, row, col, l16, av[pp], bv[pp]);
         }
 #pragma unroll
-        for (int pp = 0; pp < 2; ++pp) {
-          float sm = 0.f;
-#pragma unroll
-          for (int q = 0; q < 4; ++q) {
-            sm = __builtin_fmaf(av[pp][q].x, bv[pp][q].x, sm);
-            sm = __builtin_fmaf(av[pp][q].y, bv[pp][q].y, sm);
-            sm = __builtin_fmaf(av[pp][q].z, bv[pp][q].z, sm);
-            sm = __builtin_fmaf(av[pp][q].w, bv[pp][q].w, sm);
-          }
-          xs[h2 + pp] = row_sum16(sm);
-        }
+        for (int pp = 0; pp < 2; ++pp) xs[h2 + pp] = exact_dot16_sum(av[pp], bv[pp]);
         if (e0 + 4 * (h2 + 2) >= nlist) break;
       }
 #pragma unroll
@@ -394,13 +424,12 @@
 }
 
 hipError_t launch_screen(const void* feat0, const void* feat1, int in_dtype, int c_in, const CoarseWs& w, char* base,
-                         float inv_ct, float thr, int dense_enabled, int allow_dead, hipStream_t st) {
+                         float inv_ct, float thr, int dense_enabled, int allow_dead, bool defer, hipStream_t st) {
   ScreenArgs a;
   memset(&a, 0, sizeof(a));
   fill_screen_stats(a, w, base, inv_ct, thr, allow_dead);
-  a.in_dtype = in_dtype;
   a.q0 = w.q0.in(base); a.q1 = w.q1.in(base);
-  a.src0 = feat0; a.src1 = feat1; a.c_in = c_in;
+  a.desc = DescRows{feat0, feat1, c_in, in_dtype, w.L, w.S};
   a.rcount = w.cand.count.in(base); a.rlist_j = w.cand.idx.in(base); a.rlist_x = w.cand.x.in(base);
   a.ccount = w.ccand.count.in(base); a.clist_i = w.ccand.idx.in(base); a.clist_x = w.ccand.x.in(base);
   a.dense_enabled = dense_enabled;
@@ -411,6 +440,8 @@
   x.umax2 = w.umax2.in(base); x.upos = w.upos.in(base);
   x.look = g_unit_cert != 1;
   x.count_cert = g_unit_cert == 2;
+  x.defer = defer ? 1 : 0;
+  x.count_defer = defer && g_defer_exact == 2;
   x.chunk_units = w.units_s;
   x.nchunks = w.splits_s;
 #ifdef FM_TUNE_ENV
diff --git a/featurematching_amd/csrc/coarse_select.hip b/featurematching_amd/csrc/coarse_select.hip
--- a/featurematching_amd/csrc/coarse_select.hip
+++ b/featurematching_amd/csrc/coarse_select.hip
@@ -1,3 +1,4 @@
+#include "fm_exact_device.h"
 #include "fm_internal.h"
 #include "fm_maps_device.h"
 
@@ -14,6 +15,7 @@
   const int* cand_count_b; const int* cand_j_b; const float* cand_x_b;
   const int* ccand_count_b; const int* ccand_i_b; const float* ccand_x_b;
   const int* dense_cnt;
+  DescRows desc;
   const float* rsum; const float* csum;
   int sums_ready;
   int* blocktot; Scalars* scal;
@@ -72,6 +74,7 @@
   return pr * pc;
 }
 
+template <bool DEFER>
 __global__ __launch_bounds__(256) void k_select(SelArgs a) {
   __shared__ int sm[4];
   __shared__ int rowoff[64], rowcnt[64];
@@ -128,19 +131,34 @@
     const long g = (long)b_c * a.Lp + row;
     if (dense) return a.sums_ready ? a.rsum[g] : group_sum(share(a.rowB + (long)b_c * a.splits * a.Lp + row, a.splits, a.Lp));
     const int c2 = min(cand_count[g], a.slots);
-    const int k2 = cand_j[g * a.slots + slot];
-    const float x2 = cand_x[g * a.slots + slot];
+    const int k2t = cand_j[g * a.slots + slot];
+    const int k2 = DEFER ? (k2t & ~kDeferTag) : k2t;
+    float x2 = cand_x[g * a.slots + slot];
+    if constexpr (DEFER) {
+      bool any;
+      x2 = resolve_deferred(a.desc, b_c, slot < c2 && (k2t & kDeferTag) != 0, row, k2, x2, lane, any);
+    }
     return list_sum(__builtin_amdgcn_exp2f(__builtin_fmaf(x2, a.k, nm)), k2, slot < c2, a.slots, base, wave_max_int(c2));
   };
   const int cnt_raw = cand_count[grow_c];
-  const int j_raw = cand_j[grow_c * a.slots + slot];
-  const float x_raw = cand_x[grow_c * a.slots + slot];
+  const int j_tag = cand_j[grow_c * a.slots + slot];
+  float x_raw = cand_x[grow_c * a.slots + slot];
   const float nmr_i = a.nmr[grow_c];
   const int cnt = row_ok ? min(cnt_raw, a.slots) : 0;
   const bool live = slot < cnt;
+  const int j_raw = DEFER ? (j_tag & ~kDeferTag) : j_tag;
+  bool tag_own = DEFER && !dense && live && (j_tag & kDeferTag) != 0;
   float rs;
   if (dense) rs = a.sums_ready ? a.rsum[grow_c] : group_sum(share(a.rowB + (long)b_c * a.splits * a.Lp + i_c, a.splits, a.Lp));
-  else rs = list_sum(__builtin_amdgcn_exp2f(__builtin_fmaf(x_raw, a.k, nmr_i)), j_raw, live, a.slots, base, wave_max_int(cnt));
+  else {
+    const int maxcnt = wave_max_int(cnt);
+    if (DEFER && maxcnt > 1) {
+      bool any;
+      x_raw = resolve_deferred(a.desc, b_c, tag_own && cnt > 1, i_c, j_raw, x_raw, lane, any);
+      tag_own = tag_own && cnt == 1;
+    }
+    rs = list_sum(__builtin_amdgcn_exp2f(__builtin_fmaf(x_raw, a.k, nmr_i)), j_raw, live, a.slots, base, maxcnt);
+  }
   bool keep = false;
   int j = live ? j_raw : 0x7fffffff;
   float conf = 0.f, colbest = 0.f;
@@ -192,16 +210,32 @@
     if (!__any(t < cnt)) break;
     const bool act = t < cnt;
     const int jt = act ? __shfl(j_raw, base + t) : 0;
-    const float xt = __shfl(x_raw, base + t);
+    float xt = __shfl(x_raw, base + t);
+    bool tag_t = false;
+    if constexpr (DEFER) tag_t = !dense && act && __shfl((int)tag_own, base + t) != 0;
     const long gcol = (long)b_c * a.Sp + jt;
     const float nmc = a.nmc[gcol];
     const int ccnt = act ? min(ccand_count[gcol], a.slots) : 0;
-    const int ci = ccand_i[gcol * a.slots + slot];
-    const float cx = ccand_x[gcol * a.slots + slot];
+    const int ci_tag = ccand_i[gcol * a.slots + slot];
+    const int ci = DEFER ? (ci_tag & ~kDeferTag) : ci_tag;
+    float cx = ccand_x[gcol * a.slots + slot];
+    const bool standin = tag_t && ccnt == 1;
+    if (DEFER && !dense) {
+      bool any;
+      cx = resolve_deferred(a.desc, b_c, slot < ccnt && (ci_tag & kDeferTag) != 0 && !(standin && ci == i), ci, jt, cx, lane, any);
+      if (any) {
+        for (int e = 0; e < a.slots; ++e) {
+          const int i2 = __shfl(ci, base + e);
+          const float x2 = __shfl(cx, base + e);
+          if (tag_t && !standin && e < ccnt && i2 == i) xt = x2;
+        }
+        if (tag_t && !standin) rs = __builtin_amdgcn_exp2f(__builtin_fmaf(xt, a.k, nmr_i));
+      }
+    }
     float cs;
     if (dense) cs = a.sums_ready ? a.csum[gcol] : group_sum(share(a.colB + (long)b_c * a.panels * a.Sp + jt, a.panels, a.Sp));
     else cs = list_sum(__builtin_amdgcn_exp2f(__builtin_fmaf(cx, a.k, nmc)), ci, slot < ccnt, a.slots, base, wave_max_int(ccnt));
-    const bool col_sig = dense || __builtin_fmaf(xt, a.k, nmc) > -kSkipLog2;
+    const bool col_sig = dense || standin || __builtin_fmaf(xt, a.k, nmc) > -kSkipLog2;
     const float ct = (act && col_sig) ? entry_conf(xt, a.k, nmr_i, rs, nmc, cs) : 0.f;
     float cb = 0.f;
     const int cmax = wave_max_int(ccnt);
@@ -346,6 +380,7 @@
   a.ccand_count_b = w.ccand_b.count.in(base); a.ccand_i_b = w.ccand_b.idx.in(base);
   a.ccand_x_b = w.ccand_b.x.in(base);
   a.dense_cnt = w.dense_cnt.in(base);
+  a.desc = DescRows{c.feat0, c.feat1, c.C, c.in_dtype, w.L, w.S};
   a.rsum = w.rsum.in(base); a.csum = w.csum.in(base);
   a.blocktot = w.blocktot.in(base);
   a.scal = w.scalars.in(base);
@@ -366,7 +401,8 @@
     const long units = (long)((job->Wf + 63) / 64) * job->Hf * job->N;
     extra = (int)(units < 1024 ? units : 1024);
   }
-  hipLaunchKernelGGL(k_select, dim3(blocks + extra), dim3(256), 0, (hipStream_t)c.stream, a);
+  if (flags.deferred) hipLaunchKernelGGL(k_select<true>, dim3(blocks + extra), dim3(256), 0, (hipStream_t)c.stream, a);
+  else hipLaunchKernelGGL(k_select<false>, dim3(blocks + extra), dim3(256), 0, (hipStream_t)c.stream, a);
   return hipGetLastError();
 }
 
diff --git a/featurematching_amd/csrc/fm_debug.h b/featurematching_amd/csrc/fm_debug.h
--- a/featurematching_amd/csrc/fm_debug.h
+++ b/featurematching_amd/csrc/fm_debug.h
@@ -22,6 +22,8 @@
                          int cand_slots, float temperature, float thr, int which, void* stream);
 int fm_debug_unit_cert(int mode);
 int fm_debug_unit_cert_layout(int N, int L, int S, int C, int cand_slots, int64_t* out, int n_out);
+int fm_debug_defer_exact(int mode);
+int fm_debug_defer_exact_layout(int N, int L, int S, int C, int cand_slots, int64_t* out, int n_out);
 
 #ifdef __cplusplus
 }
diff --git a/featurematching_amd/csrc/fm_exact_device.h b/featurematching_amd/csrc/fm_exact_device.h
--- /dev/null
+++ b/featurematching_amd/csrc/fm_exact_device.h
@@ -0,0 +1,98 @@
+#pragma once
+#include "fm_device.h"
+#include "fm_wave_device.h"
+
+namespace fm {
+
+struct DescRows {
+  const void* src0; const void* src1;
+  int c_in, in_dtype, L, S;
+};
+
+__device__ __forceinline__ long desc_row0(const DescRows& d, int b, int row) { return ((long)b * d.L + row) * d.c_in; }
+__device__ __forceinline__ long desc_row1(const DescRows& d, int b, int col) { return ((long)b * d.S + col) * d.c_in; }
+
+__device__ __forceinline__ void exact_dot16_load1(const DescRows& d, long ro, long co, int l16, int q, float4& va, float4& vb) {
+  const int v4 = l16 + 16 * q;
+  const bool in = v4 < (d.c_in >> 2);
+  const int vc = in ? v4 : 0;
+  float4 ta, tb;
+  if (d.in_dtype == FM_F32) {
+    ta = reinterpret_cast<const float4*>((const float*)d.src0 + ro)[vc];
+    tb = reinterpret_cast<const float4*>((const float*)d.src1 + co)[vc];
+  } else {
+    ta = half4_to_float4(reinterpret_cast<const uint2*>((const unsigned short*)d.src0 + ro)[vc], d.in_dtype);
+    tb = half4_to_float4(reinterpret_cast<const uint2*>((const unsigned short*)d.src1 + co)[vc], d.in_dtype);
+  }
+  va = in ? ta : make_float4(0.f, 0.f, 0.f, 0.f);
+  vb = tb;
+}
+
+__device__ __forceinline__ float exact_dot16_link(float sm, const float4& va, const float4& vb) {
+  sm = __builtin_fmaf(va.x, vb.x, sm);
+  sm = __builtin_fmaf(va.y, vb.y, sm);
+  sm = __builtin_fmaf(va.z, vb.z, sm);
+  sm = __builtin_fmaf(va.w, vb.w, sm);
+  return sm;
+}
+
+__device__ __forceinline__ void exact_dot16_load(const DescRows& d, int b, int row, int col, int l16, float4 (&av)[4],
+                                                 float4 (&bv)[4]) {
+  const long ro = desc_row0(d, b, row), co = desc_row1(d, b, col);
+#pragma unroll
+  for (int q = 0; q < 4; ++q) exact_dot16_load1(d, ro, co, l16, q, av[q], bv[q]);
+}
+__device__ __forceinline__ float exact_dot16_sum(const float4 (&av)[4], const float4 (&bv)[4]) {
+  float sm = 0.f;
+#pragma unroll
+  for (int q = 0; q < 4; ++q) sm = exact_dot16_link(sm, av[q], bv[q]);
+  return row_sum16(sm);
+}
+
+__device__ __forceinline__ float exact_dot16_serial(const DescRows& d, int b, int row, int col, int l16) {
+  const long ro = desc_row0(d, b, row), co = desc_row1(d, b, col);
+  float sm = 0.f;
+#pragma nounroll
+  for (int q = 0; q < 4; ++q) {
+    float4 va, vb;
+    exact_dot16_load1(d, ro, co, l16, q, va, vb);
+    sm = exact_dot16_link(sm, va, vb);
+  }
+  return row_sum16(sm);
+}
+
+constexpr int kDeferTag = 0x40000000;
+
+__device__ __forceinline__ float resolve_deferred(const DescRows& d, int b, bool need, int row, int col, float x, int lane,
+                                                  bool& any) {
+  unsigned long long m = __ballot(need);
+  any = m != 0;
+  const int sub = lane >> 4, l16 = lane & 15;
+  while (m) {
+    int src = 0, nsrc = 0;
+    unsigned long long mm = m;
+#pragma unroll
+    for (int g = 0; g < 4; ++g) {
+      if (mm) {
+        const int l = __builtin_ctzll(mm);
+        mm &= mm - 1;
+        if (sub == g) src = l;
+        nsrc = g + 1;
+      } else if (sub == g) {
+        src = __builtin_ctzll(m);
+      }
+    }
+    const int r = __shfl(row, src), c = __shfl(col, src), bs = __shfl(b, src);
+    const float v = exact_dot16_serial(d, bs, r, c, l16);
+#pragma unroll
+    for (int g = 0; g < 4; ++g) {
+      const float vg = __shfl(v, 16 * g);
+      const int sg = __shfl(src, 16 * g);
+      if (g < nsrc && lane == sg) x = vg;
+    }
+    m = mm;
+  }
+  return x;
+}
+
+}
diff --git a/featurematching_amd/csrc/fm_internal.h b/featurematching_amd/csrc/fm_internal.h
--- a/featurematching_amd/csrc/fm_internal.h
+++ b/featurematching_amd/csrc/fm_internal.h
@@ -52,6 +52,7 @@
   unsigned flags;
   int dense_units;
   int cert_units;
+  int defer_entries;
 };
 
 struct CoarseWs {
@@ -99,6 +100,11 @@
   return g_unit_cert == 2 || (g_unit_cert == 0 && w.top2 != 0 && common_path);
 }
 
+extern int g_defer_exact;
+inline bool defer_exact_on(const CoarseWs& w, bool common_path = true) {
+  return g_defer_exact != 1 && common_path && w.Lp < 0x40000000 && w.Sp < 0x40000000;
+}
+
 struct CoarseCall {
   const void *feat0, *feat1; int in_dtype;
   int N, L, S, C, h0c, w0c, h1c, w1c;
@@ -121,14 +127,14 @@
 struct MapCopyJob {
   const float* src; float* dst; int N, Hf, Wf;
 };
-struct SelectFlags { bool exact, dense, cell_maps, sums_ready; };
+struct SelectFlags { bool exact, dense, cell_maps, sums_ready, deferred; };
 hipError_t launch_select(const CoarseWs& w, char* base, const CoarseCall& c, float inv_ct, SelectFlags flags,
                          const MapCopyJob* job = nullptr);
 hipError_t launch_conf_patch(const CoarseWs& w, char* base, float inv_ct, float* conf, hipStream_t st);
 hipError_t launch_exact_lists(const CoarseWs& w, char* base, float inv_ct, const void* feat0, const void* feat1, int in_dtype,
                               int c_in, hipStream_t st);
 hipError_t launch_screen(const void* feat0, const void* feat1, int in_dtype, int c_in, const CoarseWs& w, char* base,
-                             float inv_ct, float thr, int dense_enabled, int allow_dead, hipStream_t st);
+                             float inv_ct, float thr, int dense_enabled, int allow_dead, bool defer, hipStream_t st);
 
 struct DsmBwdWs { Span v, u, sums, part; size_t total; };
 inline DsmBwdWs dsm_bwd_layout(int N, int L, int S, int C) {
```

Measured after the change: 21200 image-pairs/s, median of 6. 1.04x the previous value.
